# jenicek/mdir

Hardware: NVIDIA B200
Metric: queries/s vs 1M x 2048 db (70-query batches, top-100, fp32-faithful ranking) (higher is better)
Workload: dtype bf16

## Files before the change

include/mdir_b200.h:

```cpp
#ifndef MDIR_B200_H
#define MDIR_B200_H

#include <stddef.h>
#include <stdint.h>

#ifdef __cplusplus
extern "C" {
#endif

#define MDIR_ABI_VERSION 3

#define MDIR_E_ARG      (-1)
#define MDIR_E_DRIVER   (-2)
#define MDIR_E_DEVICE   (-3)

int         mdir_abi_version(void);
const char* mdir_last_error(void);
int         mdir_device_check(void);
uint64_t    mdir_launch_count(void);

#define MDIR_TUNE_SCAN_MAX_CTAS 1
#define MDIR_TUNE_FINALIZE_CLUSTER 2
#define MDIR_TUNE_FINALIZE_STAGE_CAP 3
int         mdir_tune(int key, int value);

#define MDIR_POOL_GEM  0
#define MDIR_POOL_MAC  1
#define MDIR_POOL_SPOC 2
int mdir_pool(int kind, const float* x, const int64_t* off, const int32_t* hw,
              int n_maps, int C, int hw_uniform, float p, float eps,
              float* out, void* stream);

int mdir_l2n(const float* x, int N, int C, int inner, float eps, float* out, void* stream);

int mdir_ms_aggregate(const float* pooled, int n_img, int S, int C, float l2n_eps,
                      float msp, const float* m, float* out, void* stream);

int mdir_whiten_project(const float* v, const float* m, int n, int D, const float* P, int dims,
                        float renorm_eps, float* out, void* stream);

size_t mdir_whiten_tc_workspace_bytes(int n, int D, int dims);
int mdir_whiten_project_tc(const float* v, const float* m, int n, int D, const float* Px3, int dims,
                           float renorm_eps, float* out, void* ws, void* stream);

typedef struct {
    int64_t src_off;
    int64_t dst_off;
    int32_t H, W;
    int32_t src_pitch;
    int32_t dst_pitch;
} mdir_image_desc;
size_t mdir_clahe_workspace_bytes(int n_img, int tiles_x, int tiles_y);
int mdir_clahe_u8(const uint8_t* src, uint8_t* dst, const mdir_image_desc* descs,
                  int n_img, int max_H, int max_W, double clip, int tiles_x, int tiles_y,
                  void* ws, void* stream);

typedef struct {
    int64_t rgb_off;
    int64_t out_off;
    int64_t l_off;
    int32_t H, W;
} mdir_rgb_desc;
int mdir_rgb_to_l_u8(const float* rgb, const mdir_rgb_desc* descs, int n_img, int64_t max_pixels,
                     const int16_t* lut, uint8_t* l_out, void* stream);
int mdir_lab_clahe_to_rgb(const float* rgb, const mdir_rgb_desc* descs, int n_img, int64_t max_pixels,
                          const int16_t* lut, const float* gamma_tab, const uint8_t* l_in, float* out,
                          void* stream);

int mdir_pack_bf16(const float* src, int64_t n, int D, int src_is_Dxn, uint16_t* dst, void* stream);

#define MDIR_SCAN_DENSE  0
#define MDIR_SCAN_SAMPLE 1
#define MDIR_SCAN_FILTER 2
#define MDIR_SCAN_TILE_ROWS 256
#define MDIR_CAND_SEGS 149
int mdir_sim_scan_bf16(const uint16_t* db, int64_t n_db, const uint16_t* q, int n_q, int D,
                       int mode, int sample_stride, int n_sample,
                       float* dense_out, int64_t dense_ld,
                       const uint64_t* tau, uint32_t idx_base,
                       uint64_t* cand, uint32_t* seg_counts, int cap_s, int cap_l, void* stream);

int mdir_sim_scan_dense_bf16(const uint16_t* db, int64_t n_db, const uint16_t* q, int n_q, int D,
                             float* dense_out, int64_t dense_ld, void* stream);

int mdir_sim_scan_wide_bf16(const uint16_t* db, int64_t n_db, const uint16_t* q, int n_q, int D, int mode,
                            int sample_stride, int n_sample, float* dense_out, int64_t dense_ld,
                            const uint64_t* tau, uint32_t idx_base, uint64_t* cand, uint32_t* seg_counts,
                            int cap_s, int cap_l, void* stream);

size_t mdir_sim_scan_fused_workspace_bytes(int n_q);
int mdir_sim_scan_fused_bf16(const uint16_t* db, int64_t n_db, const uint16_t* q, int n_q, int D,
                             int kth, uint64_t* tau, uint32_t idx_base,
                             uint64_t* cand, uint32_t* seg_counts, int cap_s, int cap_l,
                             void* ws, void* stream);

int mdir_sim_scan_fused_i8(const int8_t* db8, const float* row_scale, int64_t n_db, const int8_t* q8,
                           const float* q_scale, int n_q, int D, int kth, uint64_t* tau, uint32_t idx_base,
                           uint64_t* cand, uint32_t* seg_counts, int cap_s, int cap_l,
                           void* ws, void* stream);

int mdir_sim_scan_tf32(const float* db, int64_t n_db, const float* q, int n_q, int D,
                       int mode, int sample_stride, int n_sample,
                       float* dense_out, int64_t dense_ld,
                       const uint64_t* tau, uint32_t idx_base,
                       uint64_t* cand, uint32_t* seg_counts, int cap_s, int cap_l, void* stream);
int mdir_split_tf32x3(const float* src, int64_t n, int D, int role, float* dst, void* stream);

int mdir_sim_scan_bf16_live(const uint16_t* db, int64_t n_db, const uint16_t* q, int n_q, int D,
                            int mode, int sample_stride, int n_sample,
                            float* dense_out, int64_t dense_ld,
                            const uint64_t* tau, uint32_t idx_base,
                            uint64_t* cand, uint32_t* seg_counts, int cap_s, int cap_l,
                            const uint32_t* live, void* stream);
int mdir_sim_scan_wide_bf16_live(const uint16_t* db, int64_t n_db, const uint16_t* q, int n_q, int D, int mode,
                                 int sample_stride, int n_sample, float* dense_out, int64_t dense_ld,
                                 const uint64_t* tau, uint32_t idx_base, uint64_t* cand, uint32_t* seg_counts,
                                 int cap_s, int cap_l, const uint32_t* live, void* stream);
int mdir_sim_scan_fused_bf16_live(const uint16_t* db, int64_t n_db, const uint16_t* q, int n_q, int D,
                                  int kth, uint64_t* tau, uint32_t idx_base,
                                  uint64_t* cand, uint32_t* seg_counts, int cap_s, int cap_l,
                                  void* ws, const uint32_t* live, void* stream);
int mdir_sim_scan_fused_i8_live(const int8_t* db8, const float* row_scale, int64_t n_db, const int8_t* q8,
                                const float* q_scale, int n_q, int D, int kth, uint64_t* tau, uint32_t idx_base,
                                uint64_t* cand, uint32_t* seg_counts, int cap_s, int cap_l,
                                void* ws, const uint32_t* live, void* stream);
int mdir_live_update(uint32_t* live, int64_t capacity, uint32_t idx_base, const int64_t* ids, int64_t n_ids,
                     int value, void* stream);

uint64_t mdir_make_key(float score, uint32_t index);
float    mdir_key_score(uint64_t key);

int mdir_select_kth(const float* scores, int64_t ld, int64_t n, int n_q, int kth,
                    int sample_stride, uint32_t idx_base,
                    uint64_t* tau, uint64_t* cand, int64_t cand_row, uint32_t* seg_counts, int n_seg,
                    int cap, int approx, void* stream);
int mdir_select_kth_live(const float* scores, int64_t ld, int64_t n, int n_q, int kth,
                         int sample_stride, uint32_t idx_base,
                         uint64_t* tau, uint64_t* cand, int64_t cand_row, uint32_t* seg_counts, int n_seg,
                         int cap, int approx, const uint32_t* live, void* stream);

int mdir_topk_finalize(const uint64_t* cand, int64_t cand_row, const uint32_t* seg_counts, int n_seg,
                       int cap0, int cap_l, int n_q, int k,
                       float* out_scores, int32_t* out_idx, uint64_t* out_keys,
                       uint64_t* tau, int32_t* overflow, void* stream);

int mdir_topk_finalize_rescore(const uint64_t* cand, int64_t cand_row, const uint32_t* seg_counts, int n_seg,
                               int cap0, int cap_l, int n_q, int shortlist, int k_out,
                               const float* db32, int64_t n_db, uint32_t idx_base, const float* q32, int D,
                               const float* db_stats,
                               float* out_scores, int32_t* out_idx, uint64_t* out_keys,
                               uint64_t* tau, int32_t* overflow, void* stream);
int mdir_topk_finalize_rescore_eps(const uint64_t* cand, int64_t cand_row, const uint32_t* seg_counts, int n_seg,
                                   int cap0, int cap_l, int n_q, int shortlist, int k_out,
                                   const float* db32, int64_t n_db, uint32_t idx_base, const float* q32, int D,
                                   const float* db_stats, const float* q_eps,
                                   float* out_scores, int32_t* out_idx, uint64_t* out_keys,
                                   uint64_t* tau, int32_t* overflow, void* stream);
#define MDIR_STATUS_OVERFLOW    1
#define MDIR_STATUS_UNCERTIFIED 2

int mdir_pack_stats(const float* db32, const uint16_t* db16, int64_t n, int D, float* stats, void* stream);

int mdir_pack_stats_i8(const float* db32, const uint16_t* db16, int64_t n, int D, float* stats,
                       int8_t* db8, float* row_scale, void* stream);

int mdir_pack_q_i8(const float* q32, int n_q, int D, const float* stats, int8_t* q8, float* q_scale,
                   float* q_eps, void* stream);

int mdir_rescore_f32(const float* db32, int64_t n_db, uint32_t idx_base, const float* q32, int n_q, int D,
                     const int32_t* idx, int kk, uint64_t* out_keys, void* stream);

int mdir_qe_accumulate(const float* db32, int64_t n_db, uint32_t idx_base, int D, const int32_t* idx,
                       const float* scores, int n_q, int n_qe, float alpha, float* acc, void* stream);
int mdir_add_l2n(const float* a, const float* b, int n, int D, float* out, void* stream);

size_t mdir_rank_workspace_bytes(int64_t n_db, int n_q);
int mdir_rank_scores(const float* scores, int64_t n_db, int n_q, int query_major,
                     int64_t* ranks, int64_t ranks_ld, void* ws, void* stream);

size_t mdir_rank_fast_workspace_bytes(int64_t n_db, int n_q);
int mdir_rank_scores_fast(const float* scores, int64_t n_db, int n_q, int query_major,
                          int64_t* ranks, int64_t ranks_ld, void* ws, int32_t* status, void* stream);

size_t mdir_rank_hist_workspace_bytes(int64_t n_db, int n_q);
int mdir_rank_scores_hist(const float* scores, int64_t n_db, int n_q, int query_major,
                          int64_t* ranks, int64_t ranks_ld, void* ws, int32_t* status, void* stream);

size_t mdir_map_workspace_bytes(int64_t n_db, int n_q);
int mdir_compute_ap(const int64_t* ranks, int64_t n_db, int n_q, const int64_t* items, const int32_t* item_query,
                    const int32_t* item_class, int64_t n_items, const int32_t* n_pos, const int32_t* kappas,
                    int n_kappa, double* aps, double* prs, void* ws, void* stream);

int mdir_topk_plan(int64_t n_db, int kth, int sm_count, int* route, int* n_sample, int* stride);
size_t mdir_sim_topk_workspace_bytes(int D);
int mdir_sim_topk_bf16(const uint16_t* db16, const float* db32, const float* db_stats, int64_t n_db,
                       const float* q32, int n_q, int D, int k, int shortlist, uint32_t idx_base, int route,
                       float* out_scores, int32_t* out_idx, uint64_t* out_keys, int32_t* overflow,
                       void* ws, void* stream);
size_t mdir_gem_head_workspace_bytes(int n_img, int S, int C, int dims);
int mdir_gem_head(int kind, const float* x, const int64_t* off, const int32_t* hw, int n_img, int S, int C,
                  int hw_uniform, float p, float eps, float msp, const float* m, const float* P,
                  const float* Px3, int dims, float* out, void* ws, void* stream);

size_t mdir_shard_mailbox_bytes(int world, int max_q, int max_k);
int mdir_p2p_alloc(size_t bytes, void** ptr, void* handle64);
int mdir_p2p_open(const void* handle64, void** ptr);
int mdir_p2p_close(void* ptr);
int mdir_p2p_free(void* ptr);
#define MDIR_EXCHANGE_SYNC 0
#define MDIR_EXCHANGE_DEFERRED 1
#define MDIR_EXCHANGE_FLUSH 2
int mdir_shard_exchange_merge(const uint64_t* local_keys, int n_q, int k, int rank, int world,
                              int max_q, int max_k, int mode, void* const* mailboxes,
                              float* out_scores, int32_t* out_idx,
                              const int32_t* local_status, int32_t* out_status, void* stream);
int mdir_shard_status(const void* own_mailbox, int* status);

int mdir_mine_negatives(const int64_t* ranks, int64_t ranks_ld, int64_t n_pool, int n_q,
                        const int32_t* pool_cluster, const int32_t* q_cluster, int nnum,
                        int64_t* out_pos, int32_t* out_found, void* stream);
int mdir_pair_l2dist(const float* q, const float* pool, const int64_t* pos, int n_q, int nnum, int D,
                     float eps, float* out, void* stream);

size_t mdir_gemm_f64_workspace_bytes(int M, int N, int64_t K);
int mdir_gemm_f64(const double* A, int64_t lda, const double* a_sub, const double* B, int64_t ldb,
                  const double* b_sub, int b_is_kxn, int M, int N, int64_t K, double alpha,
                  double* C, int64_t ldc, void* ws, void* stream);
int mdir_pair_diff_f64(const double* X, int64_t ldx, int D, int64_t n_cols, const int64_t* qidx,
                       const int64_t* pidx, int64_t n_pairs, double* out, void* stream);
int mdir_cols_mean_f64(const double* X, int64_t ldx, int D, int64_t n_cols, const int64_t* idx,
                       int64_t n_idx, double* mean, void* stream);
int mdir_f32_to_f64(const float* src, int64_t n, double* dst, void* stream);

#ifdef __cplusplus
}
#endif
#endif
```

mdir_b200/_lib.py:

```python
import ctypes as C
import os

_HERE = os.path.dirname(os.path.abspath(__file__))
LIB_PATH = os.path.join(_HERE, "libmdir_b200.so")
_lib = None
ABI_VERSION = 3


class ImageDesc(C.Structure):
    _fields_ = [("src_off", C.c_int64), ("dst_off", C.c_int64), ("H", C.c_int32), ("W", C.c_int32),
                ("src_pitch", C.c_int32), ("dst_pitch", C.c_int32)]


_vp, _i, _i64, _f, _d, _u32, _u64, _sz = C.c_void_p, C.c_int, C.c_int64, C.c_float, C.c_double, C.c_uint32, C.c_uint64, C.c_size_t

PROTOTYPES = {
    "mdir_abi_version": (_i, []),
    "mdir_last_error": (C.c_char_p, []),
    "mdir_device_check": (_i, []),
    "mdir_launch_count": (_u64, []),
    "mdir_tune": (_i, [_i, _i]),
    "mdir_pool": (_i, [_i, _vp, _vp, _vp, _i, _i, _i, _f, _f, _vp, _vp]),
    "mdir_l2n": (_i, [_vp, _i, _i, _i, _f, _vp, _vp]),
    "mdir_ms_aggregate": (_i, [_vp, _i, _i, _i, _f, _f, _vp, _vp, _vp]),
    "mdir_whiten_project": (_i, [_vp, _vp, _i, _i, _vp, _i, _f, _vp, _vp]),
    "mdir_whiten_tc_workspace_bytes": (_sz, [_i, _i, _i]),
    "mdir_whiten_project_tc": (_i, [_vp, _vp, _i, _i, _vp, _i, _f, _vp, _vp, _vp]),
    "mdir_clahe_workspace_bytes": (_sz, [_i, _i, _i]),
    "mdir_clahe_u8": (_i, [_vp, _vp, _vp, _i, _i, _i, _d, _i, _i, _vp, _vp]),
    "mdir_rgb_to_l_u8": (_i, [_vp, _vp, _i, _i64, _vp, _vp, _vp]),
    "mdir_lab_clahe_to_rgb": (_i, [_vp, _vp, _i, _i64, _vp, _vp, _vp, _vp, _vp]),
    "mdir_pack_bf16": (_i, [_vp, _i64, _i, _i, _vp, _vp]),
    "mdir_sim_scan_bf16": (_i, [_vp, _i64, _vp, _i, _i, _i, _i, _i, _vp, _i64, _vp, _u32, _vp, _vp, _i, _i, _vp]),
    "mdir_sim_scan_dense_bf16": (_i, [_vp, _i64, _vp, _i, _i, _vp, _i64, _vp]),
    "mdir_sim_scan_wide_bf16": (_i, [_vp, _i64, _vp, _i, _i, _i, _i, _i, _vp, _i64, _vp, _u32, _vp, _vp, _i, _i, _vp]),
    "mdir_sim_scan_fused_workspace_bytes": (_sz, [_i]),
    "mdir_sim_scan_fused_bf16": (_i, [_vp, _i64, _vp, _i, _i, _i, _vp, _u32, _vp, _vp, _i, _i, _vp, _vp]),
    "mdir_sim_scan_fused_i8": (_i, [_vp, _vp, _i64, _vp, _vp, _i, _i, _i, _vp, _u32, _vp, _vp, _i, _i, _vp, _vp]),
    "mdir_sim_scan_tf32": (_i, [_vp, _i64, _vp, _i, _i, _i, _i, _i, _vp, _i64, _vp, _u32, _vp, _vp, _i, _i, _vp]),
    "mdir_split_tf32x3": (_i, [_vp, _i64, _i, _i, _vp, _vp]),
    "mdir_sim_scan_bf16_live": (_i, [_vp, _i64, _vp, _i, _i, _i, _i, _i, _vp, _i64, _vp, _u32, _vp, _vp, _i, _i, _vp, _vp]),
    "mdir_sim_scan_wide_bf16_live": (_i, [_vp, _i64, _vp, _i, _i, _i, _i, _i, _vp, _i64, _vp, _u32, _vp, _vp, _i, _i, _vp, _vp]),
    "mdir_sim_scan_fused_bf16_live": (_i, [_vp, _i64, _vp, _i, _i, _i, _vp, _u32, _vp, _vp, _i, _i, _vp, _vp, _vp]),
    "mdir_sim_scan_fused_i8_live": (_i, [_vp, _vp, _i64, _vp, _vp, _i, _i, _i, _vp, _u32, _vp, _vp, _i, _i, _vp, _vp, _vp]),
    "mdir_live_update": (_i, [_vp, _i64, _u32, _vp, _i64, _i, _vp]),
    "mdir_make_key": (_u64, [_f, _u32]),
    "mdir_key_score": (_f, [_u64]),
    "mdir_select_kth": (_i, [_vp, _i64, _i64, _i, _i, _i, _u32, _vp, _vp, _i64, _vp, _i, _i, _i, _vp]),
    "mdir_select_kth_live": (_i, [_vp, _i64, _i64, _i, _i, _i, _u32, _vp, _vp, _i64, _vp, _i, _i, _i, _vp, _vp]),
    "mdir_topk_finalize": (_i, [_vp, _i64, _vp, _i, _i, _i, _i, _i, _vp, _vp, _vp, _vp, _vp, _vp]),
    "mdir_topk_finalize_rescore": (_i, [_vp, _i64, _vp, _i, _i, _i, _i, _i, _i, _vp, _i64, _u32, _vp, _i, _vp, _vp, _vp, _vp, _vp, _vp, _vp]),
    "mdir_topk_finalize_rescore_eps": (_i, [_vp, _i64, _vp, _i, _i, _i, _i, _i, _i, _vp, _i64, _u32, _vp, _i, _vp, _vp, _vp, _vp, _vp, _vp, _vp, _vp]),
    "mdir_pack_stats": (_i, [_vp, _vp, _i64, _i, _vp, _vp]),
    "mdir_pack_stats_i8": (_i, [_vp, _vp, _i64, _i, _vp, _vp, _vp, _vp]),
    "mdir_pack_q_i8": (_i, [_vp, _i, _i, _vp, _vp, _vp, _vp, _vp]),
    "mdir_rescore_f32": (_i, [_vp, _i64, _u32, _vp, _i, _i, _vp, _i, _vp, _vp]),
    "mdir_qe_accumulate": (_i, [_vp, _i64, _u32, _i, _vp, _vp, _i, _i, _f, _vp, _vp]),
    "mdir_add_l2n": (_i, [_vp, _vp, _i, _i, _vp, _vp]),
    "mdir_map_workspace_bytes": (_sz, [_i64, _i]),
    "mdir_compute_ap": (_i, [_vp, _i64, _i, _vp, _vp, _vp, _i64, _vp, _vp, _i, _vp, _vp, _vp, _vp]),
    "mdir_topk_plan": (_i, [_i64, _i, _i, _vp, _vp, _vp]),
    "mdir_sim_topk_workspace_bytes": (_sz, [_i]),
    "mdir_sim_topk_bf16": (_i, [_vp, _vp, _vp, _i64, _vp, _i, _i, _i, _i, _u32, _i, _vp, _vp, _vp, _vp, _vp, _vp]),
    "mdir_gem_head_workspace_bytes": (_sz, [_i, _i, _i, _i]),
    "mdir_gem_head": (_i, [_i, _vp, _vp, _vp, _i, _i, _i, _i, _f, _f, _f, _vp, _vp, _vp, _i, _vp, _vp, _vp]),
    "mdir_shard_mailbox_bytes": (_sz, [_i, _i, _i]),
    "mdir_p2p_alloc": (_i, [_sz, _vp, _vp]),
    "mdir_p2p_open": (_i, [_vp, _vp]),
    "mdir_p2p_close": (_i, [_vp]),
    "mdir_p2p_free": (_i, [_vp]),
    "mdir_shard_exchange_merge": (_i, [_vp, _i, _i, _i, _i, _i, _i, _i, _vp, _vp, _vp, _vp, _vp, _vp]),
    "mdir_shard_status": (_i, [_vp, _vp]),
    "mdir_mine_negatives": (_i, [_vp, _i64, _i64, _i, _vp, _vp, _i, _vp, _vp, _vp]),
    "mdir_pair_l2dist": (_i, [_vp, _vp, _vp, _i, _i, _i, _f, _vp, _vp]),
    "mdir_gemm_f64_workspace_bytes": (_sz, [_i, _i, _i64]),
    "mdir_gemm_f64": (_i, [_vp, _i64, _vp, _vp, _i64, _vp, _i, _i, _i, _i64, _d, _vp, _i64, _vp, _vp]),
    "mdir_pair_diff_f64": (_i, [_vp, _i64, _i, _i64, _vp, _vp, _i64, _vp, _vp]),
    "mdir_cols_mean_f64": (_i, [_vp, _i64, _i, _i64, _vp, _i64, _vp, _vp]),
    "mdir_f32_to_f64": (_i, [_vp, _i64, _vp, _vp]),
    "mdir_rank_workspace_bytes": (_sz, [_i64, _i]),
    "mdir_rank_scores": (_i, [_vp, _i64, _i, _i, _vp, _i64, _vp, _vp]),
    "mdir_rank_fast_workspace_bytes": (_sz, [_i64, _i]),
    "mdir_rank_scores_fast": (_i, [_vp, _i64, _i, _i, _vp, _i64, _vp, _vp, _vp]),
    "mdir_rank_hist_workspace_bytes": (_sz, [_i64, _i]),
    "mdir_rank_scores_hist": (_i, [_vp, _i64, _i, _i, _vp, _i64, _vp, _vp, _vp]),
}


class MdirError(RuntimeError):
    pass


def lib():
    global _lib
    if _lib is None:
        if not os.path.exists(LIB_PATH):
            raise MdirError("%s is missing: run `python -m mdir_b200.build` (nvcc, sm_100a). "
                            "mdir_b200 has no CPU or PyTorch fallback." % LIB_PATH)
        l = C.CDLL(LIB_PATH)
        for name, (res, args) in PROTOTYPES.items():
            fn = getattr(l, name)
            fn.restype = res
            fn.argtypes = args
        if l.mdir_abi_version() != ABI_VERSION:
            raise MdirError("libmdir_b200.so ABI mismatch")
        _lib = l
    return _lib


def check(rc, what=""):
    if rc != 0:
        msg = lib().mdir_last_error()
        raise MdirError("%s failed (code %d): %s" % (what or "libmdir_b200 call", rc, (msg or b"").decode()))


def stream():
    import torch
    return C.c_void_p(torch.cuda.current_stream().cuda_stream)


def ptr(t):
    return C.c_void_p(t.data_ptr()) if t is not None else C.c_void_p(0)


def require_cuda(t, name="tensor"):
    if not t.is_cuda:
        raise MdirError("%s must live on a CUDA device (mdir_b200 has no CPU path); got %s" % (name, t.device))
    return t
```

mdir_b200/csrc/topk.cu:

```cuda
#include <cuda_bf16.h>

#include "common.cuh"

namespace mdir {

__device__ __forceinline__ uint32_t sample_pos_to_idx(int64_t i, int sample_stride, uint32_t idx_base) {
    if (sample_stride <= 1) return idx_base + (uint32_t)i;
    const int64_t j = i / MDIR_SCAN_TILE_ROWS, r = i - j * MDIR_SCAN_TILE_ROWS;
    return idx_base + (uint32_t)(j * sample_stride * MDIR_SCAN_TILE_ROWS + r);
}

__device__ __forceinline__ bool pos_live(const uint32_t* live, int64_t i, int sample_stride) {
    if (!live) return true;
    const uint32_t r = sample_pos_to_idx(i, sample_stride, 0u);
    return (__ldg(live + (r >> 5)) >> (r & 31)) & 1u;
}

__device__ __forceinline__ uint32_t block_kth_of_thread_values(uint32_t val, uint32_t kth, uint32_t* hist, uint32_t* s_prefix,
                                                               uint32_t* s_k) {
    const int lane = threadIdx.x & 31;
    __syncthreads();
    if (threadIdx.x == 0) { *s_prefix = 0u; *s_k = kth; }
    for (int pass = 0; pass < 4; ++pass) {
        const int shift = 24 - 8 * pass;
        if (threadIdx.x < 256) hist[threadIdx.x] = 0u;
        __syncthreads();
        const uint32_t prefix = *s_prefix;
        const uint32_t himask = pass == 0 ? 0u : (0xffffffffu << (shift + 8));
        const bool hit = (val & himask) == prefix;
        if (__any_sync(0xffffffffu, hit)) {
            const int d = (int)((val >> shift) & 0xffu);
            const unsigned peers = match_digit8(d, hit);
            if (hit && lane == (__ffs(peers) - 1)) atomicAdd(&hist[d], (uint32_t)__popc(peers));
        }
        __syncthreads();
        if (threadIdx.x < 32) {
            uint32_t before;
            const int b = find_bin_warp0(hist, *s_k, &before);
            if (lane == 0) {
                *s_k -= before;
                *s_prefix = prefix | ((uint32_t)b << shift);
            }
        }
        __syncthreads();
    }
    const uint32_t r = *s_prefix;
    __syncthreads();
    return r;
}

__global__ void __launch_bounds__(1024) select_kth_kernel(const float* __restrict__ scores, int64_t ld, int64_t n, int kth,
                                                          int sample_stride, uint32_t idx_base, uint64_t* __restrict__ tau,
                                                          uint64_t* __restrict__ cand, int64_t cand_row, uint32_t* __restrict__ seg_counts,
                                                          int n_seg, int cap, const uint32_t* __restrict__ live) {
    __shared__ uint32_t hist[256];
    __shared__ uint32_t s_prefix;
    __shared__ uint32_t s_k;
    __shared__ uint32_t s_n;
    __shared__ uint32_t s_ties;
    const int q = blockIdx.x;
    const int lane = threadIdx.x & 31;
    const float* sc = scores + (int64_t)q * ld;
    uint32_t result;
    uint32_t idx_limit = 0xffffffffu;
    const int64_t n_round = (n + 8191) & ~(int64_t)8191;
    if ((int64_t)kth > n) {
        result = 0xffffffffu;
    } else {
        uint32_t bound = 0xffffffffu;
        if (kth <= 1024) {
            uint32_t mymin = 0xffffffffu;
            for (int64_t base = 0; base < n_round; base += 8 * 1024) {
                float v[8];
#pragma unroll
                for (int u = 0; u < 8; ++u) {
                    const int64_t i = base + u * 1024 + threadIdx.x;
                    v[u] = i < n ? __ldg(sc + i) : 0.f;
                }
#pragma unroll
                for (int u = 0; u < 8; ++u) {
                    const int64_t i = base + u * 1024 + threadIdx.x;
                    if (i < n && pos_live(live, i, sample_stride)) mymin = min(mymin, desc_key(v[u]));
                }
            }
            bound = block_kth_of_thread_values(mymin, (uint32_t)kth, hist, &s_prefix, &s_k);
        }
        if (threadIdx.x == 0) { s_prefix = 0u; s_k = (uint32_t)kth; }
        for (int pass = 0; pass < 4; ++pass) {
            const int shift = 24 - 8 * pass;
            if (threadIdx.x < 256) hist[threadIdx.x] = 0u;
            __syncthreads();
            const uint32_t prefix = s_prefix;
            const uint32_t himask = pass == 0 ? 0u : (0xffffffffu << (shift + 8));
            for (int64_t base = 0; base < n_round; base += 8 * 1024) {
                float v[8];
#pragma unroll
                for (int u = 0; u < 8; ++u) {
                    const int64_t i = base + u * 1024 + threadIdx.x;
                    v[u] = i < n ? __ldg(sc + i) : 0.f;
                }
#pragma unroll
                for (int u = 0; u < 8; ++u) {
                    const int64_t i = base + u * 1024 + threadIdx.x;
                    const bool valid = i < n && pos_live(live, i, sample_stride);
                    const uint32_t key = desc_key(v[u]);
                    const bool hit = valid && key <= bound && ((key & himask) == prefix);
                    if (__any_sync(0xffffffffu, hit)) {
                        const int d = (int)((key >> shift) & 0xffu);
                        const unsigned peers = match_digit8(d, hit);
                        if (hit && lane == (__ffs(peers) - 1)) atomicAdd(&hist[d], (uint32_t)__popc(peers));
                    }
                }
            }
            __syncthreads();
            if (threadIdx.x < 32) {
                uint32_t before;
                const int b = find_bin_warp0(hist, s_k, &before);
                if (lane == 0) {
                    s_k -= before;
                    s_prefix = prefix | ((uint32_t)b << shift);
                    s_ties = hist[b];
                }
            }
            __syncthreads();
        }
        result = s_prefix;
        if (s_k < s_ties) {
            __syncthreads();
            if (threadIdx.x == 0) s_prefix = 0u;
            for (int pass = 0; pass < 4; ++pass) {
                const int shift = 24 - 8 * pass;
                if (threadIdx.x < 256) hist[threadIdx.x] = 0u;
                __syncthreads();
                const uint32_t prefix = s_prefix;
                const uint32_t himask = pass == 0 ? 0u : (0xffffffffu << (shift + 8));
                for (int64_t base = 0; base < n_round; base += 1024) {
                    const int64_t i = base + threadIdx.x;
                    const bool valid = i < n && pos_live(live, i, sample_stride);
                    const float v = valid ? __ldg(sc + i) : 0.f;
                    const uint32_t idx = sample_pos_to_idx(valid ? i : 0, sample_stride, idx_base);
                    const bool hit = valid && (desc_key(v) == result) && ((idx & himask) == prefix);
                    if (__any_sync(0xffffffffu, hit)) {
                        const int d = (int)((idx >> shift) & 0xffu);
                        const unsigned peers = match_digit8(d, hit);
                        if (hit && lane == (__ffs(peers) - 1)) atomicAdd(&hist[d], (uint32_t)__popc(peers));
                    }
                }
                __syncthreads();
                if (threadIdx.x < 32) {
                    uint32_t before;
                    const int b = find_bin_warp0(hist, s_k, &before);
                    if (lane == 0) {
                        s_k -= before;
                        s_prefix = prefix | ((uint32_t)b << shift);
                    }
                }
                __syncthreads();
            }
            idx_limit = s_prefix;
        }
    }
    const uint64_t tau_key = ((uint64_t)result << 32) | (uint64_t)idx_limit;
    __syncthreads();
    if (threadIdx.x == 0) { tau[q] = tau_key; s_n = 0u; }
    if (cand) {
        __syncthreads();
        for (int64_t base = 0; base < n_round; base += 8 * 1024) {
            float v[8];
#pragma unroll
            for (int u = 0; u < 8; ++u) {
                const int64_t i = base + u * 1024 + threadIdx.x;
                v[u] = i < n ? __ldg(sc + i) : -INFINITY;
            }
#pragma unroll
            for (int u = 0; u < 8; ++u) {
                const int64_t i = base + u * 1024 + threadIdx.x;
                if (i < n && desc_key(v[u]) <= result && pos_live(live, i, sample_stride)) {
                    const uint64_t key = make_key(v[u], sample_pos_to_idx(i, sample_stride, idx_base));
                    if (key <= tau_key) {
                        const uint32_t pos = atomicAdd(&s_n, 1u);
                        if (pos < (uint32_t)cap) cand[(int64_t)q * cand_row + pos] = key;
                    }
                }
            }
        }
        __syncthreads();
        if (threadIdx.x == 0) seg_counts[(int64_t)q * n_seg] = s_n;
        for (int sg = 1 + threadIdx.x; sg < n_seg; sg += blockDim.x) seg_counts[(int64_t)q * n_seg + sg] = 0u;
    }
}

__global__ void __launch_bounds__(1024, 1) select_kth_reg_kernel(const float* __restrict__ scores, int64_t ld, int n, int kth,
                                                                 int sample_stride, uint32_t idx_base, uint64_t* __restrict__ tau,
                                                                 uint64_t* __restrict__ cand, int64_t cand_row,
                                                                 uint32_t* __restrict__ seg_counts, int n_seg, int cap, int approx,
                                                                 const uint32_t* __restrict__ live) {
    __shared__ uint32_t hist[256];
    __shared__ uint32_t s_prefix, s_k, s_n, s_ties;
    const int q = blockIdx.x;
    const int lane = threadIdx.x & 31;
    const float* sc = scores + (int64_t)q * ld;
    uint32_t key[32];
#pragma unroll
    for (int u = 0; u < 32; ++u) {
        const int i = u * 1024 + threadIdx.x;
        key[u] = i < n && pos_live(live, i, sample_stride) ? desc_key(__ldg(sc + i)) : 0xffffffffu;
    }
    auto valid = [&](int u) { return live ? key[u] != 0xffffffffu : u * 1024 + (int)threadIdx.x < n; };
    uint32_t result = 0xffffffffu, idx_limit = 0xffffffffu;
    if (kth <= n) {
        uint32_t bound = 0xffffffffu;
        if (kth <= 1024) {
            uint32_t mymin = 0xffffffffu;
#pragma unroll
            for (int u = 0; u < 32; ++u)
                if (valid(u)) mymin = min(mymin, key[u]);
            bound = block_kth_of_thread_values(mymin, (uint32_t)kth, hist, &s_prefix, &s_k);
        }
        const bool use_bound = approx && kth <= 1024;
        if (threadIdx.x == 0) { s_prefix = use_bound ? bound : 0u; s_k = use_bound ? 0u : (uint32_t)kth; s_ties = 0u; }
        if (use_bound) __syncthreads();
        for (int pass = 0; pass < (use_bound ? 0 : 4); ++pass) {
            const int shift = 24 - 8 * pass;
            if (threadIdx.x < 256) hist[threadIdx.x] = 0u;
            __syncthreads();
            const uint32_t prefix = s_prefix;
            const uint32_t himask = pass == 0 ? 0u : (0xffffffffu << (shift + 8));
#pragma unroll
            for (int u = 0; u < 32; ++u) {
                const bool hit = valid(u) && key[u] <= bound && ((key[u] & himask) == prefix);
                if (__any_sync(0xffffffffu, hit)) {
                    const int d = (int)((key[u] >> shift) & 0xffu);
                    const unsigned peers = match_digit8(d, hit);
                    if (hit && lane == (__ffs(peers) - 1)) atomicAdd(&hist[d], (uint32_t)__popc(peers));
                }
            }
            __syncthreads();
            if (threadIdx.x < 32) {
                uint32_t before;
                const int b = find_bin_warp0(hist, s_k, &before);
                if (lane == 0) {
                    s_k -= before;
                    s_prefix = prefix | ((uint32_t)b << shift);
                    s_ties = hist[b];
                }
            }
            __syncthreads();
        }
        result = s_prefix;
        if (s_k < s_ties) {
            __syncthreads();
            if (threadIdx.x == 0) s_prefix = 0u;
            for (int pass = 0; pass < 4; ++pass) {
                const int shift = 24 - 8 * pass;
                if (threadIdx.x < 256) hist[threadIdx.x] = 0u;
                __syncthreads();
                const uint32_t prefix = s_prefix;
                const uint32_t himask = pass == 0 ? 0u : (0xffffffffu << (shift + 8));
#pragma unroll
                for (int u = 0; u < 32; ++u) {
                    const int i = u * 1024 + threadIdx.x;
                    const uint32_t idx = sample_pos_to_idx(i, sample_stride, idx_base);
                    const bool hit = valid(u) && key[u] == result && ((idx & himask) == prefix);
                    if (__any_sync(0xffffffffu, hit)) {
                        const int d = (int)((idx >> shift) & 0xffu);
                        const unsigned peers = match_digit8(d, hit);
                        if (hit && lane == (__ffs(peers) - 1)) atomicAdd(&hist[d], (uint32_t)__popc(peers));
                    }
                }
                __syncthreads();
                if (threadIdx.x < 32) {
                    uint32_t before;
                    const int b = find_bin_warp0(hist, s_k, &before);
                    if (lane == 0) {
                        s_k -= before;
                        s_prefix = prefix | ((uint32_t)b << shift);
                    }
                }
                __syncthreads();
            }
            idx_limit = s_prefix;
        }
    }
    const uint64_t tau_key = ((uint64_t)result << 32) | (uint64_t)idx_limit;
    __syncthreads();
    if (threadIdx.x == 0) { tau[q] = tau_key; s_n = 0u; }
    if (cand) {
        __syncthreads();
#pragma unroll
        for (int u = 0; u < 32; ++u) {
            const int i = u * 1024 + threadIdx.x;
            if (valid(u) && key[u] <= result) {
                const uint64_t k64 = ((uint64_t)key[u] << 32) | (uint64_t)sample_pos_to_idx(i, sample_stride, idx_base);
                if (k64 <= tau_key) {
                    const uint32_t pos = atomicAdd(&s_n, 1u);
                    if (pos < (uint32_t)cap) cand[(int64_t)q * cand_row + pos] = k64;
                }
            }
        }
        __syncthreads();
        if (threadIdx.x == 0) seg_counts[(int64_t)q * n_seg] = s_n;
        for (int sg = 1 + threadIdx.x; sg < n_seg; sg += blockDim.x) seg_counts[(int64_t)q * n_seg + sg] = 0u;
    }
}

__device__ __forceinline__ uint32_t cluster_ctarank() {
    uint32_t r;
    asm volatile("mov.u32 %0, %%cluster_ctarank;" : "=r"(r));
    return r;
}
__device__ __forceinline__ void cluster_sync_all() {
    asm volatile("barrier.cluster.arrive.release.aligned;\n\tbarrier.cluster.wait.acquire.aligned;" ::: "memory");
}
__device__ __forceinline__ uint32_t cluster_map(const void* p, uint32_t rank) {
    const uint32_t a = (uint32_t)__cvta_generic_to_shared(p);
    uint32_t r;
    asm volatile("mapa.shared::cluster.u32 %0, %1, %2;" : "=r"(r) : "r"(a), "r"(rank));
    return r;
}
__device__ __forceinline__ uint64_t cluster_ld_u64(uint32_t a) {
    uint64_t v;
    asm volatile("ld.shared::cluster.u64 %0, [%1];" : "=l"(v) : "r"(a) : "memory");
    return v;
}
__device__ __forceinline__ void cluster_st_u64(uint32_t a, uint64_t v) {
    asm volatile("st.shared::cluster.u64 [%0], %1;" ::"r"(a), "l"(v) : "memory");
}
__device__ __forceinline__ int cluster_ld_s32(uint32_t a) {
    int v;
    asm volatile("ld.shared::cluster.s32 %0, [%1];" : "=r"(v) : "r"(a) : "memory");
    return v;
}

__device__ __forceinline__ float rescore_row(const float* __restrict__ a, const float* qs, int D, int lane) {
    float acc = 0.f;
    if ((D & 3) == 0) {
        const float4* a4 = reinterpret_cast<const float4*>(a);
        const float4* b4 = reinterpret_cast<const float4*>(qs);
        const int n4 = D >> 2;
        float acc1 = 0.f, acc2 = 0.f, acc3 = 0.f;
        int i = lane;
        for (; i + 96 < n4; i += 128) {
            const float4 x0 = __ldg(a4 + i), x1 = __ldg(a4 + i + 32), x2 = __ldg(a4 + i + 64), x3 = __ldg(a4 + i + 96);
            const float4 y0 = b4[i], y1 = b4[i + 32], y2 = b4[i + 64], y3 = b4[i + 96];
            acc = fmaf(x0.x, y0.x, acc); acc = fmaf(x0.y, y0.y, acc); acc = fmaf(x0.z, y0.z, acc); acc = fmaf(x0.w, y0.w, acc);
            acc1 = fmaf(x1.x, y1.x, acc1); acc1 = fmaf(x1.y, y1.y, acc1); acc1 = fmaf(x1.z, y1.z, acc1); acc1 = fmaf(x1.w, y1.w, acc1);
            acc2 = fmaf(x2.x, y2.x, acc2); acc2 = fmaf(x2.y, y2.y, acc2); acc2 = fmaf(x2.z, y2.z, acc2); acc2 = fmaf(x2.w, y2.w, acc2);
            acc3 = fmaf(x3.x, y3.x, acc3); acc3 = fmaf(x3.y, y3.y, acc3); acc3 = fmaf(x3.z, y3.z, acc3); acc3 = fmaf(x3.w, y3.w, acc3);
        }
        for (; i < n4; i += 32) {
            const float4 x = __ldg(a4 + i), y = b4[i];
            acc = fmaf(x.x, y.x, acc); acc = fmaf(x.y, y.y, acc); acc = fmaf(x.z, y.z, acc); acc = fmaf(x.w, y.w, acc);
        }
        acc = (acc + acc1) + (acc2 + acc3);
    } else {
        for (int i = lane; i < D; i += 32) acc = fmaf(a[i], qs[i], acc);
    }
    return warp_sum(acc);
}

__device__ __forceinline__ bool topk_hist_select(uint64_t* skeys, int cnt, int k, int kpow2, uint64_t* out, uint32_t* hist, uint32_t* s_n,
                                                 uint32_t* scratch) {
    const int lane = threadIdx.x & 31, w = threadIdx.x >> 5;
    uint32_t mn = 0xffffffffu, mx = 0u;
    for (int i = threadIdx.x; i < cnt; i += blockDim.x) {
        const uint32_t h = (uint32_t)(skeys[i] >> 32);
        mn = min(mn, h);
        mx = max(mx, h);
    }
    mn = __reduce_min_sync(0xffffffffu, mn);
    mx = __reduce_max_sync(0xffffffffu, mx);
    if (lane == 0) { scratch[w] = mn; scratch[32 + w] = mx; }
    hist[threadIdx.x] = 0u;
    if (threadIdx.x == 0) *s_n = 0u;
    __syncthreads();
    mn = scratch[lane];
    mx = scratch[32 + lane];
    mn = __reduce_min_sync(0xffffffffu, mn);
    mx = __reduce_max_sync(0xffffffffu, mx);
    const float scale = 1024.0f / ((float)(mx - mn) + 1.0f);
    auto bin_of = [&](uint64_t key) { return min(1023, (int)((float)((uint32_t)(key >> 32) - mn) * scale)); };
    for (int i = threadIdx.x; i < cnt; i += blockDim.x) atomicAdd(&hist[bin_of(skeys[i])], 1u);
    __syncthreads();
    const uint32_t c = hist[threadIdx.x];
    uint32_t incl = c;
#pragma unroll
    for (int o = 1; o < 32; o <<= 1) {
        const uint32_t t = __shfl_up_sync(0xffffffffu, incl, o);
        if (lane >= o) incl += t;
    }
    __syncthreads();
    if (lane == 31) scratch[w] = incl;
    __syncthreads();
    uint32_t pre = 0;
    for (int j = 0; j < w; ++j) pre += scratch[j];
    incl += pre;
    if (incl >= (uint32_t)k && incl - c < (uint32_t)k) { scratch[32] = threadIdx.x; scratch[33] = incl; }
    if (threadIdx.x == 1023 && incl < (uint32_t)k) { scratch[32] = 1023u; scratch[33] = incl; }
    __syncthreads();
    const int b_star = (int)scratch[32];
    const int take = (int)scratch[33];
    if (take > 1024) return false;
    uint64_t* sel = skeys + cnt;
    for (int i = threadIdx.x; i < cnt; i += blockDim.x) {
        const uint64_t key = skeys[i];
        if (bin_of(key) <= b_star) sel[atomicAdd(s_n, 1u)] = key;
    }
    for (int i = threadIdx.x; i < kpow2; i += blockDim.x) out[i] = ~0ull;
    __syncthreads();
    if ((int)threadIdx.x < take) {
        const uint64_t mine = sel[threadIdx.x];
        int r = 0;
        for (int j = 0; j < take; ++j) r += sel[j] < mine ? 1 : 0;
        if (r < kpow2) out[r] = mine;
    }
    __syncthreads();
    return true;
}

__device__ __forceinline__ void rescore_row2(const float* __restrict__ a0, const float* __restrict__ a1, const float* qs, int D, int lane,
                                             float& r0, float& r1) {
    if ((D & 3) != 0) {
        r0 = rescore_row(a0, qs, D, lane);
        r1 = rescore_row(a1, qs, D, lane);
        return;
    }
    const float4* p0 = reinterpret_cast<const float4*>(a0);
    const float4* p1 = reinterpret_cast<const float4*>(a1);
    const float4* b4 = reinterpret_cast<const float4*>(qs);
    const int n4 = D >> 2;
    float s0a = 0.f, s0b = 0.f, s1a = 0.f, s1b = 0.f;
    int i = lane;
    for (; i + 96 < n4; i += 128) {
        const float4 x0 = __ldg(p0 + i), x1 = __ldg(p0 + i + 32), x2 = __ldg(p0 + i + 64), x3 = __ldg(p0 + i + 96);
        const float4 z0 = __ldg(p1 + i), z1 = __ldg(p1 + i + 32), z2 = __ldg(p1 + i + 64), z3 = __ldg(p1 + i + 96);
        float4 y = b4[i];
        s0a = fmaf(x0.x, y.x, s0a); s0a = fmaf(x0.y, y.y, s0a); s0a = fmaf(x0.z, y.z, s0a); s0a = fmaf(x0.w, y.w, s0a);
        s1a = fmaf(z0.x, y.x, s1a); s1a = fmaf(z0.y, y.y, s1a); s1a = fmaf(z0.z, y.z, s1a); s1a = fmaf(z0.w, y.w, s1a);
        y = b4[i + 32];
        s0b = fmaf(x1.x, y.x, s0b); s0b = fmaf(x1.y, y.y, s0b); s0b = fmaf(x1.z, y.z, s0b); s0b = fmaf(x1.w, y.w, s0b);
        s1b = fmaf(z1.x, y.x, s1b); s1b = fmaf(z1.y, y.y, s1b); s1b = fmaf(z1.z, y.z, s1b); s1b = fmaf(z1.w, y.w, s1b);
        y = b4[i + 64];
        s0a = fmaf(x2.x, y.x, s0a); s0a = fmaf(x2.y, y.y, s0a); s0a = fmaf(x2.z, y.z, s0a); s0a = fmaf(x2.w, y.w, s0a);
        s1a = fmaf(z2.x, y.x, s1a); s1a = fmaf(z2.y, y.y, s1a); s1a = fmaf(z2.z, y.z, s1a); s1a = fmaf(z2.w, y.w, s1a);
        y = b4[i + 96];
        s0b = fmaf(x3.x, y.x, s0b); s0b = fmaf(x3.y, y.y, s0b); s0b = fmaf(x3.z, y.z, s0b); s0b = fmaf(x3.w, y.w, s0b);
        s1b = fmaf(z3.x, y.x, s1b); s1b = fmaf(z3.y, y.y, s1b); s1b = fmaf(z3.z, y.z, s1b); s1b = fmaf(z3.w, y.w, s1b);
    }
    for (; i < n4; i += 32) {
        const float4 x = __ldg(p0 + i), z = __ldg(p1 + i), y = b4[i];
        s0a = fmaf(x.x, y.x, s0a); s0a = fmaf(x.y, y.y, s0a); s0a = fmaf(x.z, y.z, s0a); s0a = fmaf(x.w, y.w, s0a);
        s1a = fmaf(z.x, y.x, s1a); s1a = fmaf(z.y, y.y, s1a); s1a = fmaf(z.z, y.z, s1a); s1a = fmaf(z.w, y.w, s1a);
    }
    r0 = warp_sum(s0a + s0b);
    r1 = warp_sum(s1a + s1b);
}

template <int CS>
__device__ __forceinline__ void rescore_share(uint64_t* local_list, uint32_t remote_list, bool remote, int j0, int n, int crank,
                                              const float* __restrict__ db32, int64_t n_db, uint32_t idx_base, const float* qs, int D) {
    const int lane = threadIdx.x & 31;
    for (int j = (threadIdx.x >> 5) * CS + crank; j < n; j += 64 * CS) {
        const int jb = j + 32 * CS;
        const uint64_t key0 = remote ? cluster_ld_u64(remote_list + 8u * (uint32_t)(j0 + j)) : local_list[j0 + j];
        uint64_t key1 = ~0ull;
        if (jb < n) key1 = remote ? cluster_ld_u64(remote_list + 8u * (uint32_t)(j0 + jb)) : local_list[j0 + jb];
        const uint32_t g0 = (uint32_t)key0, g1 = (uint32_t)key1;
        const int64_t row0 = (int64_t)g0 - (int64_t)idx_base, row1 = (int64_t)g1 - (int64_t)idx_base;
        const bool ok0 = key0 != ~0ull && row0 >= 0 && row0 < n_db, ok1 = key1 != ~0ull && row1 >= 0 && row1 < n_db;
        float s0 = 0.f, s1 = 0.f;
        if (ok0 && ok1) rescore_row2(db32 + row0 * D, db32 + row1 * D, qs, D, lane, s0, s1);
        else if (ok0) s0 = rescore_row(db32 + row0 * D, qs, D, lane);
        else if (ok1) s1 = rescore_row(db32 + row1 * D, qs, D, lane);
        const uint64_t n0 = ok0 ? make_key(s0, g0) : ~0ull, n1 = ok1 ? make_key(s1, g1) : ~0ull;
        __syncwarp();
        if (lane == 0) {
            if (remote) {
                cluster_st_u64(remote_list + 8u * (uint32_t)(j0 + j), n0);
                if (jb < n) cluster_st_u64(remote_list + 8u * (uint32_t)(j0 + jb), n1);
            } else {
                local_list[j0 + j] = n0;
                if (jb < n) local_list[j0 + jb] = n1;
            }
        }
    }
}

template <int CS>
__global__ void __launch_bounds__(1024) topk_finalize_kernel(const uint64_t* __restrict__ cand, int64_t cand_row,
                                                             const uint32_t* __restrict__ seg_counts, int n_seg, int cap0, int cap_l,
                                                             int k, int smem_cap, int sl_cap, float* __restrict__ out_scores,
                                                             int32_t* __restrict__ out_idx, uint64_t* __restrict__ out_keys,
                                                             uint64_t* __restrict__ tau, int32_t* __restrict__ overflow,
                                                             const float* __restrict__ db32, int64_t n_db, uint32_t idx_base,
                                                             const float* __restrict__ q32, int D, int k_out,
                                                             const float* __restrict__ db_stats, const float* __restrict__ q_eps) {
    extern __shared__ uint64_t skeys[];
    __shared__ uint32_t hist[256];
    __shared__ uint64_t s_prefix;
    __shared__ uint32_t s_k, s_done, s_out;
    __shared__ int s_off[MDIR_CAND_SEGS + 1];
    __shared__ int s_ovf;
    __shared__ int s_hdr[3];
    __shared__ uint64_t s_tkey;
    __shared__ float s_red[96];
    __shared__ uint32_t hist_sel[1024];
    uint64_t* sorted = skeys + smem_cap;
    const int q = blockIdx.x / CS;
    const int crank = CS > 1 ? (int)cluster_ctarank() : 0;
    const int lane = threadIdx.x & 31;
    int kpow2 = 32;
    while (kpow2 < k) kpow2 <<= 1;
    if (CS > 1 && crank != 0) {
        float* qs = reinterpret_cast<float*>(sorted + sl_cap);
        for (int i = threadIdx.x; i < D; i += blockDim.x) qs[i] = q32[(int64_t)q * D + i];
        __syncthreads();
        cluster_sync_all();
        const int nk = cluster_ld_s32(cluster_map(&s_hdr[0], 0));
        const int off = cluster_ld_s32(cluster_map(&s_hdr[1], 0));
        const uint32_t rk0 = cluster_map(skeys + off, 0);
        rescore_share<CS>(nullptr, rk0, true, 0, nk, crank, db32, n_db, idx_base, qs, D);
        cluster_sync_all();
        cluster_sync_all();
        const int n_ext = cluster_ld_s32(cluster_map(&s_hdr[2], 0));
        rescore_share<CS>(nullptr, rk0, true, nk, n_ext, crank, db32, n_db, idx_base, qs, D);
        cluster_sync_all();
        return;
    }
    const uint64_t tau_in = tau ? tau[q] : ~0ull;
    if (threadIdx.x < 32) {
        constexpr int kRounds = (MDIR_CAND_SEGS + 31) / 32;
        uint32_t raw[kRounds];
#pragma unroll
        for (int i = 0; i < kRounds; ++i) {
            const int sg = i * 32 + lane;
            raw[i] = sg < n_seg ? seg_counts[(int64_t)q * n_seg + sg] : 0u;
        }
        int run = 0, ovf = 0;
#pragma unroll
        for (int i = 0; i < kRounds; ++i) {
            const int sg = i * 32 + lane;
            int c = 0;
            if (sg < n_seg) {
                const uint32_t cp = (uint32_t)(sg == 0 ? cap0 : cap_l);
                if (raw[i] > cp) ovf = 1;
                c = (int)min(raw[i], cp);
            }
            int incl = c;
#pragma unroll
            for (int o = 1; o < 32; o <<= 1) {
                const int t = __shfl_up_sync(0xffffffffu, incl, o);
                if (lane >= o) incl += t;
            }
            if (sg < n_seg) s_off[sg] = run + incl - c;
            run += __shfl_sync(0xffffffffu, incl, 31);
        }
        ovf = __any_sync(0xffffffffu, ovf);
        if (lane == 0) { s_off[n_seg] = run; s_ovf = ovf; }
    }
    __syncthreads();
    const int total = s_off[n_seg];
    const int cnt = min(total, smem_cap);
    const bool ovf_any = s_ovf || total > smem_cap;
    {
        const uint64_t* row = cand + (int64_t)q * cand_row;
        for (int p = threadIdx.x; p < cnt; p += blockDim.x) {
            int lo = 0, hi = n_seg;
            while (hi - lo > 1) {
                const int mid = (lo + hi) >> 1;
                if (s_off[mid] <= p) lo = mid; else hi = mid;
            }
            const int64_t base = lo == 0 ? 0 : (int64_t)cap0 + (int64_t)(lo - 1) * cap_l;
            skeys[p] = row[base + (p - s_off[lo])];
        }
    }
    __syncthreads();
    const uint64_t* res;
    int nres;
    if (cnt > k + 96 && cnt + 1024 <= smem_cap &&
        topk_hist_select(skeys, cnt, k, kpow2, sorted, hist_sel, &s_out, reinterpret_cast<uint32_t*>(s_red))) {
        res = sorted;
        nres = min(cnt, k);
    } else if (cnt <= 1024 && cnt + kpow2 <= smem_cap) {
        uint64_t mine = ~0ull;
        int r = 0;
        if ((int)threadIdx.x < cnt) {
            mine = skeys[threadIdx.x];
            for (int j = 0; j < cnt; ++j) r += skeys[j] < mine ? 1 : 0;
        }
        __syncthreads();
        if ((int)threadIdx.x < cnt) skeys[r] = mine;
        for (int i = cnt + threadIdx.x; i < cnt + kpow2 && i < smem_cap; i += blockDim.x) skeys[i] = ~0ull;
        __syncthreads();
        res = skeys;
        nres = cnt;
    } else if (cnt <= 2 * kpow2 || cnt <= 1024) {
        int n = 32;
        while (n < cnt) n <<= 1;
        for (int i = cnt + threadIdx.x; i < n; i += blockDim.x) skeys[i] = ~0ull;
        __syncthreads();
        bitonic_sort_smem(skeys, n);
        res = skeys;
        nres = cnt;
    } else {
        if (threadIdx.x == 0) { s_prefix = 0ull; s_k = (uint32_t)k; s_done = 0u; s_out = 0u; }
        __syncthreads();
        const int cnt_round = (cnt + 1023) & ~1023;
        uint64_t thresh = ~0ull;
        for (int pass = 0; pass < 8; ++pass) {
            const int shift = 56 - 8 * pass;
            if (threadIdx.x < 256) hist[threadIdx.x] = 0u;
            __syncthreads();
            const uint64_t prefix = s_prefix;
            const uint64_t himask = pass == 0 ? 0ull : (~0ull << (shift + 8));
            for (int i = threadIdx.x; i < cnt_round; i += 1024) {
                const bool valid = i < cnt;
                const uint64_t key = valid ? skeys[i] : 0ull;
                const bool hit = valid && ((key & himask) == prefix);
                if (__any_sync(0xffffffffu, hit)) {
                    const int d = (int)((key >> shift) & 0xffu);
                    const unsigned peers = match_digit8(d, hit);
                    if (hit && lane == (__ffs(peers) - 1)) atomicAdd(&hist[d], (uint32_t)__popc(peers));
                }
            }
            __syncthreads();
            if (threadIdx.x < 32) {
                uint32_t before;
                const int b = find_bin_warp0(hist, s_k, &before);
                if (lane == 0) {
                    const uint32_t need = s_k - before;
                    s_k = need;
                    s_prefix = prefix | ((uint64_t)b << shift);
                    if (need == hist[b] || shift == 0) s_done = 1u;
                }
            }
            __syncthreads();
            if (s_done) {
                thresh = s_prefix | (shift ? ((1ull << shift) - 1ull) : 0ull);
                break;
            }
        }
        for (int i = threadIdx.x; i < kpow2; i += blockDim.x) sorted[i] = ~0ull;
        __syncthreads();
        for (int i = threadIdx.x; i < cnt; i += blockDim.x) {
            const uint64_t key = skeys[i];
            if (key <= thresh) {
                const uint32_t pos = atomicAdd(&s_out, 1u);
                if (pos < (uint32_t)kpow2) sorted[pos] = key;
            }
        }
        __syncthreads();
        bitonic_sort_smem(sorted, kpow2);
        res = sorted;
        nres = min(cnt, k);
    }
    int status = ovf_any ? 1 : 0;
    if (threadIdx.x == 0 && ovf_any && tau && nres > 0) tau[q] = res[min(k, nres) - 1];
    int k_emit = k;
    if (db32) {
        uint64_t* sl = sorted;
        float* qs = reinterpret_cast<float*>(sorted + sl_cap);
        const int nk = min(k, nres);
        if (res != sl) {
            for (int j = threadIdx.x; j < nk; j += blockDim.x) sl[j] = res[j];
        }
        float q2 = 0.f, qt2 = 0.f, qf2 = 0.f;
        for (int i = threadIdx.x; i < D; i += blockDim.x) {
            const float v = q32[(int64_t)q * D + i];
            qs[i] = v;
            const float vt = __bfloat162float(__float2bfloat16_rn(v));
            q2 = fmaf(v, v, q2);
            qt2 = fmaf(vt, vt, qt2);
            qf2 = fmaf(v - vt, v - vt, qf2);
        }
        if (threadIdx.x == 0) { s_hdr[0] = nk; s_hdr[1] = (int)(sl - skeys); s_hdr[2] = 0; s_out = 0u; s_tkey = ~0ull; }
        __syncthreads();
        const uint64_t last16 = nk > 0 ? sl[nk - 1] : 0ull;
        float eps = 0.f;
        if (db_stats && q_eps) {
            eps = q_eps[q];
        } else if (db_stats) {
            q2 = warp_sum(q2); qt2 = warp_sum(qt2); qf2 = warp_sum(qf2);
            const int wi = threadIdx.x >> 5;
            if (lane == 0) { s_red[wi] = q2; s_red[32 + wi] = qt2; s_red[64 + wi] = qf2; }
            __syncthreads();
            q2 = warp_sum(s_red[lane]); qt2 = warp_sum(s_red[32 + lane]); qf2 = warp_sum(s_red[64 + lane]);
            const float e_max = sqrtf(db_stats[0]), x_max = sqrtf(db_stats[1]);
            eps = e_max * sqrtf(qt2) + x_max * sqrtf(qf2) + 1.25f * (float)D * 5.9604645e-8f * x_max * sqrtf(q2);
            eps = eps * 1.001f + 1e-7f;
        }
        __syncthreads();
        if (CS > 1) cluster_sync_all();
        rescore_share<CS>(sl, 0u, false, 0, nk, 0, db32, n_db, idx_base, qs, D);
        if (CS > 1) cluster_sync_all();
        __syncthreads();
        int n_ext = 0;
        if (db_stats) {
            if (nk >= k_out) {
                if (nk <= 1024) {
                    if ((int)threadIdx.x < nk) {
                        const uint64_t mine = sl[threadIdx.x];
                        int r = 0;
                        for (int j = 0; j < nk; ++j) {
                            const uint64_t o = sl[j];
                            r += (o < mine || (o == mine && j < (int)threadIdx.x)) ? 1 : 0;
                        }
                        if (r == k_out - 1) s_tkey = mine;
                    }
                } else {
                    for (int j = nk + threadIdx.x; j < kpow2; j += blockDim.x) sl[j] = ~0ull;
                    __syncthreads();
                    bitonic_sort_smem(sl, kpow2);
                    if (threadIdx.x == 0) s_tkey = sl[k_out - 1];
                }
            }
            __syncthreads();
            const uint64_t tkey = s_tkey;
            const uint64_t bound = tkey == ~0ull ? ~0ull : ((uint64_t)desc_key(key_score(tkey) - eps) << 32) | 0xffffffffull;
            const int ext_cap = sl_cap - nk;
            for (int i = threadIdx.x; i < cnt; i += blockDim.x) {
                const uint64_t key = skeys[i];
                if (key > last16 && key <= bound && key != ~0ull) {
                    const uint32_t pos = atomicAdd(&s_out, 1u);
                    if (pos < (uint32_t)ext_cap) sl[nk + pos] = key;
                }
            }
            __syncthreads();
            n_ext = min((int)s_out, ext_cap);
            if ((int)s_out > ext_cap || bound > tau_in || ovf_any) status |= 2;
            if (threadIdx.x == 0) s_hdr[2] = n_ext;
            __syncthreads();
        }
        if (CS > 1) cluster_sync_all();
        rescore_share<CS>(sl, 0u, false, nk, n_ext, 0, db32, n_db, idx_base, qs, D);
        if (CS > 1) cluster_sync_all();
        __syncthreads();
        const int n_all = nk + n_ext;
        if (n_all <= 1024) {
            if ((int)threadIdx.x < n_all) {
                const uint64_t mine = sl[threadIdx.x];
                int r = 0;
                for (int j = 0; j < n_all; ++j) {
                    const uint64_t o = sl[j];
                    r += (o < mine || (o == mine && j < (int)threadIdx.x)) ? 1 : 0;
                }
                skeys[r] = mine;
            }
            __syncthreads();
            res = skeys;
        } else {
            int n = 32;
            while (n < n_all) n <<= 1;
            for (int j = n_all + threadIdx.x; j < n; j += blockDim.x) sl[j] = ~0ull;
            __syncthreads();
            bitonic_sort_smem(sl, n);
            res = sl;
        }
        nres = n_all;
        k_emit = k_out;
    }
    if (threadIdx.x == 0 && overflow) overflow[q] = status;
    for (int j = threadIdx.x; j < k_emit; j += blockDim.x) {
        const uint64_t key = j < nres ? res[j] : ~0ull;
        const bool ok = j < nres && key != ~0ull;
        if (out_scores) out_scores[(int64_t)q * k_emit + j] = ok ? key_score(key) : -INFINITY;
        if (out_idx) out_idx[(int64_t)q * k_emit + j] = ok ? (int32_t)(uint32_t)key : -1;
        if (out_keys) out_keys[(int64_t)q * k_emit + j] = ok ? key : ~0ull;
    }
}

__global__ void __launch_bounds__(256) rescore_f32_kernel(const float* __restrict__ db32, int64_t n_db, uint32_t idx_base,
                                                          const float* __restrict__ q32, int n_q, int D,
                                                          const int32_t* __restrict__ idx, int kk, uint64_t* __restrict__ out_keys) {
    const int lane = threadIdx.x & 31;
    const int64_t item = (int64_t)blockIdx.x * (blockDim.x >> 5) + (threadIdx.x >> 5);
    if (item >= (int64_t)n_q * kk) return;
    const int q = (int)(item / kk);
    const int32_t gi = idx[item];
    const int64_t row = (int64_t)(uint32_t)gi - (int64_t)idx_base;
    if (gi < 0 || row < 0 || row >= n_db) {
        if (lane == 0) out_keys[item] = ~0ull;
        return;
    }
    const float* a = db32 + row * D;
    const float* b = q32 + (int64_t)q * D;
    float acc = 0.f;
    if ((D & 3) == 0) {
        const float4* a4 = reinterpret_cast<const float4*>(a);
        const float4* b4 = reinterpret_cast<const float4*>(b);
        for (int i = lane; i < (D >> 2); i += 32) {
            const float4 x = a4[i], y = b4[i];
            acc = fmaf(x.x, y.x, acc); acc = fmaf(x.y, y.y, acc); acc = fmaf(x.z, y.z, acc); acc = fmaf(x.w, y.w, acc);
        }
    } else {
        for (int i = lane; i < D; i += 32) acc = fmaf(a[i], b[i], acc);
    }
    acc = warp_sum(acc);
    if (lane == 0) out_keys[item] = make_key(acc, (uint32_t)gi);
}

__global__ void __launch_bounds__(256) pack_bf16_rows_kernel(const float* __restrict__ src, int64_t total, __nv_bfloat16* __restrict__ dst) {
    const int64_t i = ((int64_t)blockIdx.x * blockDim.x + threadIdx.x) * 4;
    if (i + 3 < total) {
        const float4 v = *reinterpret_cast<const float4*>(src + i);
        __nv_bfloat162 lo = __floats2bfloat162_rn(v.x, v.y), hi = __floats2bfloat162_rn(v.z, v.w);
        uint2 o;
        o.x = *reinterpret_cast<uint32_t*>(&lo);
        o.y = *reinterpret_cast<uint32_t*>(&hi);
        *reinterpret_cast<uint2*>(dst + i) = o;
    } else {
        for (int64_t j = i; j < total; ++j) dst[j] = __float2bfloat16_rn(src[j]);
    }
}

__global__ void __launch_bounds__(256) pack_bf16_transpose_kernel(const float* __restrict__ src, int64_t n, int D,
                                                                  __nv_bfloat16* __restrict__ dst) {
    __shared__ float tile[32][33];
    const int64_t n0 = (int64_t)blockIdx.x * 32;
    const int d0 = blockIdx.y * 32;
    const int tx = threadIdx.x & 31, ty = threadIdx.x >> 5;
    for (int r = ty; r < 32; r += 8) {
        const int d = d0 + r;
        const int64_t i = n0 + tx;
        tile[r][tx] = (d < D && i < n) ? src[(int64_t)d * n + i] : 0.f;
    }
    __syncthreads();
    for (int r = ty; r < 32; r += 8) {
        const int64_t i = n0 + r;
        const int d = d0 + tx;
        if (i < n && d < D) dst[i * D + d] = __float2bfloat16_rn(tile[tx][r]);
    }
}

__global__ void __launch_bounds__(256) qe_accumulate_kernel(const float* __restrict__ db32, int64_t n_db, uint32_t idx_base, int D,
                                                            const int32_t* __restrict__ idx, const float* __restrict__ scores,
                                                            int n_qe, float alpha, float* __restrict__ acc) {
    __shared__ float w_s[256];
    __shared__ int64_t row_s[256];
    const int q = blockIdx.x;
    for (int j = threadIdx.x; j < n_qe; j += blockDim.x) {
        const int32_t gi = idx[(int64_t)q * n_qe + j];
        const int64_t row = (int64_t)(uint32_t)gi - (int64_t)idx_base;
        const bool own = gi >= 0 && row >= 0 && row < n_db;
        row_s[j] = own ? row : -1;
        w_s[j] = own ? powf(fmaxf(scores[(int64_t)q * n_qe + j], 0.f), alpha) : 0.f;
    }
    __syncthreads();
    for (int d = threadIdx.x; d < D; d += blockDim.x) {
        float a = 0.f;
        for (int j = 0; j < n_qe; ++j)
            if (row_s[j] >= 0) a = fmaf(w_s[j], db32[row_s[j] * D + d], a);
        acc[(int64_t)q * D + d] = a;
    }
}

__global__ void __launch_bounds__(256) add_l2n_kernel(const float* a, const float* b, int D, float* out) {
    __shared__ float red[32];
    const int n = blockIdx.x;
    float s = 0.f;
    for (int d = threadIdx.x; d < D; d += blockDim.x) {
        const float v = a[(int64_t)n * D + d] + (b ? b[(int64_t)n * D + d] : 0.f);
        s += v * v;
    }
    s = block_sum(s, red);
    const float inv = 1.0f / sqrtf(s);
    for (int d = threadIdx.x; d < D; d += blockDim.x)
        out[(int64_t)n * D + d] = (a[(int64_t)n * D + d] + (b ? b[(int64_t)n * D + d] : 0.f)) * inv;
}

}

using namespace mdir;

extern "C" uint64_t mdir_make_key(float score, uint32_t index) { return make_key(score, index); }
extern "C" float mdir_key_score(uint64_t key) { return key_score(key); }

extern "C" int mdir_select_kth_live(const float* scores, int64_t ld, int64_t n, int n_q, int kth, int sample_stride,
                                    uint32_t idx_base, uint64_t* tau, uint64_t* cand, int64_t cand_row, uint32_t* seg_counts, int n_seg,
                                    int cap, int approx, const uint32_t* live, void* stream) {
    MDIR_CHECK_ARG(scores && tau && n >= 0 && n_q >= 0 && kth >= 1 && ld >= n);
    MDIR_CHECK_ARG(cand == nullptr || (seg_counts != nullptr && cap >= 1 && n_seg >= 1 && cand_row >= cap));
    if (n_q == 0) return 0;
    if (n <= 32 * 1024) {
        select_kth_reg_kernel<<<n_q, 1024, 0, (cudaStream_t)stream>>>(scores, ld, (int)n, kth, sample_stride, idx_base, tau, cand,
                                                                      cand_row, seg_counts, n_seg, cap, approx, live);
        MDIR_LAUNCH_CHECK();
        return 0;
    }
    select_kth_kernel<<<n_q, 1024, 0, (cudaStream_t)stream>>>(scores, ld, n, kth, sample_stride, idx_base, tau, cand, cand_row,
                                                              seg_counts, n_seg, cap, live);
    MDIR_LAUNCH_CHECK();
    return 0;
}

extern "C" int mdir_select_kth(const float* scores, int64_t ld, int64_t n, int n_q, int kth, int sample_stride,
                               uint32_t idx_base, uint64_t* tau, uint64_t* cand, int64_t cand_row, uint32_t* seg_counts, int n_seg,
                               int cap, int approx, void* stream) {
    return mdir_select_kth_live(scores, ld, n, n_q, kth, sample_stride, idx_base, tau, cand, cand_row, seg_counts, n_seg, cap, approx,
                                nullptr, stream);
}

namespace mdir {
__global__ void __launch_bounds__(256) live_update_kernel(uint32_t* __restrict__ live, int64_t capacity, uint32_t idx_base,
                                                          const int64_t* __restrict__ ids, int64_t n_ids, int value) {
    const int64_t i = (int64_t)blockIdx.x * blockDim.x + threadIdx.x;
    if (i >= n_ids) return;
    const int64_t r = ids[i] - (int64_t)idx_base;
    if (r < 0 || r >= capacity) return;
    const uint32_t bit = 1u << (uint32_t)(r & 31);
    if (value) atomicOr(live + (r >> 5), bit);
    else atomicAnd(live + (r >> 5), ~bit);
}
}

extern "C" int mdir_live_update(uint32_t* live, int64_t capacity, uint32_t idx_base, const int64_t* ids, int64_t n_ids, int value,
                                void* stream) {
    MDIR_CHECK_ARG(live && capacity >= 0 && n_ids >= 0 && (ids || n_ids == 0));
    if (n_ids == 0) return 0;
    MDIR_CHECK_ARG((n_ids + 255) / 256 <= 0x7fffffff);
    live_update_kernel<<<(unsigned)((n_ids + 255) / 256), 256, 0, (cudaStream_t)stream>>>(live, capacity, idx_base, ids, n_ids, value);
    MDIR_LAUNCH_CHECK();
    return 0;
}

static int launch_finalize(const uint64_t* cand, int64_t cand_row, const uint32_t* seg_counts, int n_seg, int cap0, int cap_l, int n_q,
                           int k, float* out_scores, int32_t* out_idx, uint64_t* out_keys, uint64_t* tau, int32_t* overflow,
                           const float* db32, int64_t n_db, uint32_t idx_base, const float* q32, int D, int k_out, const float* db_stats,
                           void* stream, const float* q_eps = nullptr) {
    MDIR_CHECK_ARG(cand && seg_counts && n_seg >= 1 && n_seg <= MDIR_CAND_SEGS && cap0 >= 0 && n_q >= 0 && k >= 1 && k <= 4096);
    MDIR_CHECK_ARG(n_seg == 1 || cap_l >= 1);
    MDIR_CHECK_ARG(cand_row >= (int64_t)cap0 + (int64_t)(n_seg - 1) * cap_l);
    if (n_q == 0) return 0;
    int kpow2 = 32;
    while (kpow2 < k) kpow2 <<= 1;
    int64_t want = (int64_t)cap0 + (int64_t)(n_seg - 1) * cap_l;
    int smem_cap = 1024;
    while (smem_cap < want && smem_cap < 16384) smem_cap <<= 1;
    if (g_finalize_stage_cap > 0 && smem_cap > g_finalize_stage_cap) smem_cap = g_finalize_stage_cap;
    if (smem_cap < 2 * kpow2) smem_cap = 2 * kpow2;
    int sl_cap = db32 ? 2 * kpow2 : kpow2;
    if (db32 && q_eps) {
        const int64_t want = (int64_t)kpow2 + n_db / 512;
        while (sl_cap < want && sl_cap < 2048) sl_cap <<= 1;
    }
    size_t smem = (size_t)(smem_cap + sl_cap) * 8;
    if (db32) {
        MDIR_CHECK_ARG(q32 && D > 0 && D <= 8192 && k_out >= 1 && k_out <= k && n_db >= 0);
        MDIR_CHECK_ARG((((uintptr_t)db32 | (uintptr_t)q32) & 15) == 0);
        MDIR_CHECK_ARG(db_stats == nullptr || tau != nullptr);
        smem += (size_t)D * 4;
    }
    constexpr int kFinalizeMaxSmem = 232448 - 7424;
    MDIR_CHECK_ARG(smem <= (size_t)kFinalizeMaxSmem);
    static PerDeviceOnce once;
    if (once.first() != 0) {
        const int max_smem = kFinalizeMaxSmem;
        MDIR_CUDA(cudaFuncSetAttribute(topk_finalize_kernel<1>, cudaFuncAttributeMaxDynamicSharedMemorySize, max_smem));
        MDIR_CUDA(cudaFuncSetAttribute(topk_finalize_kernel<2>, cudaFuncAttributeMaxDynamicSharedMemorySize, max_smem));
    }
    const int sm_count = device_sm_count();
    if (db32 && g_finalize_cluster && 2 * n_q <= sm_count) {
        cudaLaunchConfig_t cfg = {};
        cfg.gridDim = dim3(2 * n_q);
        cfg.blockDim = dim3(1024);
        cfg.dynamicSmemBytes = smem;
        cfg.stream = (cudaStream_t)stream;
        cudaLaunchAttribute attr[1];
        attr[0].id = cudaLaunchAttributeClusterDimension;
        attr[0].val.clusterDim.x = 2;
        attr[0].val.clusterDim.y = 1;
        attr[0].val.clusterDim.z = 1;
        cfg.attrs = attr;
        cfg.numAttrs = 1;
        MDIR_CUDA(cudaLaunchKernelEx(&cfg, topk_finalize_kernel<2>, cand, cand_row, seg_counts, n_seg, cap0, cap_l, k, smem_cap, sl_cap, out_scores,
                                     out_idx, out_keys, tau, overflow, db32, n_db, idx_base, q32, D, k_out, db_stats, q_eps));
        MDIR_LAUNCH_CHECK();
        return 0;
    }
    topk_finalize_kernel<1><<<n_q, 1024, smem, (cudaStream_t)stream>>>(cand, cand_row, seg_counts, n_seg, cap0, cap_l, k, smem_cap, sl_cap,
                                                                        out_scores, out_idx, out_keys, tau, overflow, db32, n_db, idx_base,
                                                                        q32, D, k_out, db_stats, q_eps);
    MDIR_LAUNCH_CHECK();
    return 0;
}

extern "C" int mdir_topk_finalize(const uint64_t* cand, int64_t cand_row, const uint32_t* seg_counts, int n_seg, int cap0, int cap_l,
                                  int n_q, int k, float* out_scores, int32_t* out_idx, uint64_t* out_keys, uint64_t* tau,
                                  int32_t* overflow, void* stream) {
    return launch_finalize(cand, cand_row, seg_counts, n_seg, cap0, cap_l, n_q, k, out_scores, out_idx, out_keys, tau, overflow, nullptr, 0,
                           0, nullptr, 0, 0, nullptr, stream);
}

extern "C" int mdir_topk_finalize_rescore(const uint64_t* cand, int64_t cand_row, const uint32_t* seg_counts, int n_seg, int cap0,
                                          int cap_l, int n_q, int shortlist, int k_out, const float* db32, int64_t n_db,
                                          uint32_t idx_base, const float* q32, int D, const float* db_stats, float* out_scores,
                                          int32_t* out_idx, uint64_t* out_keys, uint64_t* tau, int32_t* overflow, void* stream) {
    MDIR_CHECK_ARG(db32 != nullptr);
    return launch_finalize(cand, cand_row, seg_counts, n_seg, cap0, cap_l, n_q, shortlist, out_scores, out_idx, out_keys, tau, overflow,
                           db32, n_db, idx_base, q32, D, k_out, db_stats, stream);
}

extern "C" int mdir_topk_finalize_rescore_eps(const uint64_t* cand, int64_t cand_row, const uint32_t* seg_counts, int n_seg, int cap0,
                                              int cap_l, int n_q, int shortlist, int k_out, const float* db32, int64_t n_db,
                                              uint32_t idx_base, const float* q32, int D, const float* db_stats, const float* q_eps,
                                              float* out_scores, int32_t* out_idx, uint64_t* out_keys, uint64_t* tau, int32_t* overflow,
                                              void* stream) {
    MDIR_CHECK_ARG(db32 != nullptr && db_stats != nullptr && q_eps != nullptr);
    return launch_finalize(cand, cand_row, seg_counts, n_seg, cap0, cap_l, n_q, shortlist, out_scores, out_idx, out_keys, tau, overflow,
                           db32, n_db, idx_base, q32, D, k_out, db_stats, stream, q_eps);
}

namespace mdir {
__global__ void __launch_bounds__(256) pack_stats_kernel(const float* __restrict__ db32, const __nv_bfloat16* __restrict__ db16, int64_t n, int D,
                                                         uint32_t* __restrict__ stats) {
    const int lane = threadIdx.x & 31;
    const int64_t warps = (int64_t)gridDim.x * (blockDim.x >> 5);
    float e_max = 0.f, x_max = 0.f;
    for (int64_t r = (int64_t)blockIdx.x * (blockDim.x >> 5) + (threadIdx.x >> 5); r < n; r += warps) {
        const float* a = db32 + r * D;
        const __nv_bfloat16* b = db16 + r * D;
        float e2 = 0.f, x2 = 0.f;
        for (int i = lane; i < D; i += 32) {
            const float x = a[i];
            const float d = __bfloat162float(b[i]) - x;
            e2 = fmaf(d, d, e2);
            x2 = fmaf(x, x, x2);
        }
        e_max = fmaxf(e_max, warp_sum(e2));
        x_max = fmaxf(x_max, warp_sum(x2));
    }
    if (lane == 0) {
        atomicMax(&stats[0], __float_as_uint(e_max * 1.0001f));
        atomicMax(&stats[1], __float_as_uint(x_max * 1.0001f));
    }
}
}

extern "C" int mdir_pack_stats(const float* db32, const uint16_t* db16, int64_t n, int D, float* stats, void* stream) {
    MDIR_CHECK_ARG(db32 && db16 && stats && n >= 0 && D > 0);
    MDIR_CUDA(cudaMemsetAsync(stats, 0, 2 * sizeof(float), (cudaStream_t)stream));
    if (n == 0) return 0;
    const int64_t blocks = (n + 7) / 8;
    pack_stats_kernel<<<(unsigned)(blocks < 148 * 8 ? blocks : 148 * 8), 256, 0, (cudaStream_t)stream>>>(
        db32, reinterpret_cast<const __nv_bfloat16*>(db16), n, D, reinterpret_cast<uint32_t*>(stats));
    MDIR_LAUNCH_CHECK();
    return 0;
}

namespace mdir {
__device__ __forceinline__ float quant_i8(float v, float s) {
    return s > 0.f ? fminf(fmaxf(rintf(__fdiv_rn(v, s)), -127.f), 127.f) : 0.f;
}

__global__ void __launch_bounds__(256) pack_stats_i8_kernel(const float* __restrict__ db32, const __nv_bfloat16* __restrict__ db16, int64_t n,
                                                            int D, uint32_t* __restrict__ stats, int8_t* __restrict__ db8,
                                                            float* __restrict__ row_scale) {
    const int lane = threadIdx.x & 31;
    const int64_t warps = (int64_t)gridDim.x * (blockDim.x >> 5);
    float e_max = 0.f, x_max = 0.f, e8_max = 0.f, rel_max = 0.f;
    for (int64_t r = (int64_t)blockIdx.x * (blockDim.x >> 5) + (threadIdx.x >> 5); r < n; r += warps) {
        const float* a = db32 + r * D;
        const __nv_bfloat16* b = db16 + r * D;
        float e2 = 0.f, x2 = 0.f, m = 0.f;
        for (int i = lane; i < D; i += 32) {
            const float x = a[i];
            const float d = __bfloat162float(b[i]) - x;
            e2 = fmaf(d, d, e2);
            x2 = fmaf(x, x, x2);
            m = fmaxf(m, fabsf(x));
        }
        e2 = warp_sum(e2);
        x2 = warp_sum(x2);
        const float s = __fdiv_rn(warp_max(m), 127.f);
        float q2 = 0.f;
        for (int i = lane * 4; i < D; i += 128) {
            const float4 x = *reinterpret_cast<const float4*>(a + i);
            const float c0 = quant_i8(x.x, s), c1 = quant_i8(x.y, s), c2 = quant_i8(x.z, s), c3 = quant_i8(x.w, s);
            char4 o;
            o.x = (signed char)c0; o.y = (signed char)c1; o.z = (signed char)c2; o.w = (signed char)c3;
            *reinterpret_cast<char4*>(db8 + r * D + i) = o;
            const float d0 = fmaf(-s, c0, x.x), d1 = fmaf(-s, c1, x.y), d2 = fmaf(-s, c2, x.z), d3 = fmaf(-s, c3, x.w);
            q2 = fmaf(d0, d0, fmaf(d1, d1, fmaf(d2, d2, fmaf(d3, d3, q2))));
        }
        q2 = warp_sum(q2);
        if (lane == 0) row_scale[r] = s;
        e_max = fmaxf(e_max, e2);
        x_max = fmaxf(x_max, x2);
        e8_max = fmaxf(e8_max, q2);
        if (x2 > 0.f) rel_max = fmaxf(rel_max, q2 / x2);
    }
    if (lane == 0) {
        atomicMax(&stats[0], __float_as_uint(e_max * 1.0001f));
        atomicMax(&stats[1], __float_as_uint(x_max * 1.0001f));
        atomicMax(&stats[2], __float_as_uint(e8_max * 1.001f));
        atomicMax(&stats[3], __float_as_uint(rel_max * 1.001f));
    }
}

__global__ void __launch_bounds__(32) pack_q_i8_kernel(const float* __restrict__ q32, int n_q, int n_pad, int D, const float* __restrict__ stats,
                                                       int8_t* __restrict__ q8, float* __restrict__ q_scale, float* __restrict__ q_eps) {
    const int q = blockIdx.x, lane = threadIdx.x;
    int8_t* hi_row = q8 + (int64_t)q * D;
    int8_t* lo_row = q8 + (int64_t)(n_pad + q) * D;
    if (q >= n_q) {
        for (int i = lane * 4; i < D; i += 128) {
            *reinterpret_cast<char4*>(hi_row + i) = make_char4(0, 0, 0, 0);
            *reinterpret_cast<char4*>(lo_row + i) = make_char4(0, 0, 0, 0);
        }
        return;
    }
    const float* v = q32 + (int64_t)q * D;
    float m = 0.f, q2 = 0.f;
    for (int i = lane; i < D; i += 32) {
        const float x = v[i];
        m = fmaxf(m, fabsf(x));
        q2 = fmaf(x, x, q2);
    }
    const float s_hi = __fdiv_rn(warp_max(m), 127.f);
    float m2 = 0.f;
    for (int i = lane; i < D; i += 32) m2 = fmaxf(m2, fabsf(fmaf(-s_hi, quant_i8(v[i], s_hi), v[i])));
    const float s_lo = __fdiv_rn(warp_max(m2), 127.f);
    float h2 = 0.f, l2 = 0.f, qh2 = 0.f, d2 = 0.f;
    for (int i = lane * 4; i < D; i += 128) {
        const float4 x = *reinterpret_cast<const float4*>(v + i);
        const float xs[4] = {x.x, x.y, x.z, x.w};
        signed char ho[4], lo[4];
#pragma unroll
        for (int j = 0; j < 4; ++j) {
            const float h = quant_i8(xs[j], s_hi);
            const float r = fmaf(-s_hi, h, xs[j]);
            const float l = quant_i8(r, s_lo);
            const float d = fmaf(-s_lo, l, r);
            const float qh = fmaf(s_lo, l, s_hi * h);
            ho[j] = (signed char)h;
            lo[j] = (signed char)l;
            h2 = fmaf(h, h, h2);
            l2 = fmaf(l, l, l2);
            qh2 = fmaf(qh, qh, qh2);
            d2 = fmaf(d, d, d2);
        }
        *reinterpret_cast<char4*>(hi_row + i) = make_char4(ho[0], ho[1], ho[2], ho[3]);
        *reinterpret_cast<char4*>(lo_row + i) = make_char4(lo[0], lo[1], lo[2], lo[3]);
    }
    q2 = warp_sum(q2); h2 = warp_sum(h2); l2 = warp_sum(l2); qh2 = warp_sum(qh2); d2 = warp_sum(d2);
    if (lane == 0) {
        const float x_max = sqrtf(stats[1]), e8 = sqrtf(stats[2]);
        const float u = 5.9604645e-8f;
        float eps = e8 * sqrtf(qh2) + x_max * sqrtf(d2) + 1.25f * (float)D * u * x_max * sqrtf(q2) +
                    8.f * u * (x_max + e8) * (s_hi * sqrtf(h2) + s_lo * sqrtf(l2));
        q_scale[2 * q] = s_hi;
        q_scale[2 * q + 1] = s_lo;
        q_eps[q] = eps * 1.001f + 1e-7f;
    }
}
}

extern "C" int mdir_pack_stats_i8(const float* db32, const uint16_t* db16, int64_t n, int D, float* stats, int8_t* db8, float* row_scale,
                                  void* stream) {
    MDIR_CHECK_ARG(db32 && db16 && stats && db8 && row_scale && n >= 0 && D > 0 && D % 128 == 0);
    MDIR_CHECK_ARG((((uintptr_t)db32 | (uintptr_t)db8) & 15) == 0);
    MDIR_CUDA(cudaMemsetAsync(stats, 0, 4 * sizeof(float), (cudaStream_t)stream));
    if (n == 0) return 0;
    const int64_t blocks = (n + 7) / 8;
    pack_stats_i8_kernel<<<(unsigned)(blocks < 148 * 8 ? blocks : 148 * 8), 256, 0, (cudaStream_t)stream>>>(
        db32, reinterpret_cast<const __nv_bfloat16*>(db16), n, D, reinterpret_cast<uint32_t*>(stats), db8, row_scale);
    MDIR_LAUNCH_CHECK();
    return 0;
}

extern "C" int mdir_pack_q_i8(const float* q32, int n_q, int D, const float* stats, int8_t* q8, float* q_scale, float* q_eps, void* stream) {
    MDIR_CHECK_ARG(q32 && stats && q8 && q_scale && q_eps && n_q >= 1 && n_q <= 128 && D > 0 && D % 128 == 0);
    MDIR_CHECK_ARG((((uintptr_t)q32 | (uintptr_t)q8) & 15) == 0);
    const int n_pad = (n_q + 15) & ~15;
    pack_q_i8_kernel<<<n_pad, 32, 0, (cudaStream_t)stream>>>(q32, n_q, n_pad, D, stats, q8, q_scale, q_eps);
    MDIR_LAUNCH_CHECK();
    return 0;
}

extern "C" int mdir_rescore_f32(const float* db32, int64_t n_db, uint32_t idx_base, const float* q32, int n_q, int D,
                                const int32_t* idx, int kk, uint64_t* out_keys, void* stream) {
    MDIR_CHECK_ARG(db32 && q32 && idx && out_keys && n_db >= 0 && n_q >= 0 && D > 0 && kk >= 1);
    MDIR_CHECK_ARG((((uintptr_t)db32 | (uintptr_t)q32) & 15) == 0);
    const int64_t items = (int64_t)n_q * kk;
    if (items == 0) return 0;
    rescore_f32_kernel<<<(unsigned)((items + 7) / 8), 256, 0, (cudaStream_t)stream>>>(db32, n_db, idx_base, q32, n_q, D, idx, kk,
                                                                                      out_keys);
    MDIR_LAUNCH_CHECK();
    return 0;
}

extern "C" int mdir_pack_bf16(const float* src, int64_t n, int D, int src_is_Dxn, uint16_t* dst, void* stream) {
    MDIR_CHECK_ARG(src && dst && n >= 0 && D > 0);
    if (n == 0) return 0;
    cudaStream_t st = (cudaStream_t)stream;
    if (!src_is_Dxn) {
        MDIR_CHECK_ARG((((uintptr_t)src & 15) | ((uintptr_t)dst & 7)) == 0);
        const int64_t total = n * D;
        const int64_t threads = (total + 3) / 4;
        pack_bf16_rows_kernel<<<(unsigned)((threads + 255) / 256), 256, 0, st>>>(src, total, (__nv_bfloat16*)dst);
    } else {
        dim3 grid((unsigned)((n + 31) / 32), (unsigned)((D + 31) / 32));
        MDIR_CHECK_ARG(grid.y <= 65535);
        pack_bf16_transpose_kernel<<<grid, 256, 0, st>>>(src, n, D, (__nv_bfloat16*)dst);
    }
    MDIR_LAUNCH_CHECK();
    return 0;
}

extern "C" int mdir_qe_accumulate(const float* db32, int64_t n_db, uint32_t idx_base, int D, const int32_t* idx, const float* scores,
                                  int n_q, int n_qe, float alpha, float* acc, void* stream) {
    MDIR_CHECK_ARG(db32 && idx && scores && acc && n_db >= 0 && D > 0 && n_q >= 0 && n_qe >= 1 && n_qe <= 256);
    if (n_q == 0) return 0;
    qe_accumulate_kernel<<<n_q, 256, 0, (cudaStream_t)stream>>>(db32, n_db, idx_base, D, idx, scores, n_qe, alpha, acc);
    MDIR_LAUNCH_CHECK();
    return 0;
}

extern "C" int mdir_add_l2n(const float* a, const float* b, int n, int D, float* out, void* stream) {
    MDIR_CHECK_ARG(a && out && n >= 0 && D > 0);
    if (n == 0) return 0;
    add_l2n_kernel<<<n, 256, 0, (cudaStream_t)stream>>>(a, b, D, out);
    MDIR_LAUNCH_CHECK();
    return 0;
}
```

mdir_b200/search.py:

```python
import contextlib

import numpy as np
import torch

from . import _lib

TILE = 256
MAX_Q = 128
DENSE_LAUNCH_Q = 1 << 20
MAX_Q_WIDE = 256
SINGLE_GPU_SCAN_CTAS = 140
WIDE_Q = 1024
N_SEGS = 149
CAP_S = 8192
CAP_L = 96
CAND_ROW = CAP_S + 148 * CAP_L
STAGE_CAP = 16384
MAX_SAMPLE_TILES = 512
FUSED_CAP_L = CAND_ROW // 148
TARGET_CAND = 4500


STATUS_OVERFLOW, STATUS_UNCERTIFIED, STATUS_PEER_TIMEOUT = 1, 2, 4
MAX_KTH = 4096
I8_MAX_REL_RESIDUAL = 0.02
I8_MIN_ROWS = 900000


def default_shortlist(k):
    return -(-(-(-5 * int(k) // 4)) // 64) * 64


def balanced_grid(n_work, max_ctas):
    if n_work <= 0 or max_ctas <= 0:
        return 1
    if n_work <= max_ctas:
        return int(n_work)
    rounds = -(-n_work // max_ctas)
    return int(-(-n_work // rounds))


def _as_dev_f32(x, device):
    if isinstance(x, np.ndarray):
        x = torch.from_numpy(np.ascontiguousarray(x, dtype=np.float32))
    if x.dtype != torch.float32:
        x = x.float()
    if x.device != device:
        x = x.pin_memory().to(device, non_blocking=True) if x.device.type == "cpu" else x.to(device)
    return x.contiguous()


def pack_bf16(x, dxn=False, out=None):
    _lib.require_cuda(x, "descriptors")
    x = x.contiguous()
    if dxn:
        D, n = x.shape
    else:
        n, D = x.shape
    if D % 8:
        raise _lib.MdirError("descriptor dimension must be a multiple of 8 (got %d)" % D)
    if out is None:
        out = torch.empty((n, D), dtype=torch.bfloat16, device=x.device)
    with torch.cuda.device(x.device):
        _lib.check(_lib.lib().mdir_pack_bf16(_lib.ptr(x), n, D, 1 if dxn else 0, _lib.ptr(out), _lib.stream()), "mdir_pack_bf16")
    return out


def check_ids(ids, lo, hi):
    if isinstance(ids, torch.Tensor):
        ids = ids.detach().cpu().numpy()
    a = np.asarray(ids)
    if a.size and not np.issubdtype(a.dtype, np.integer):
        raise _lib.MdirError("ids must be integers (got %s)" % a.dtype)
    a = a.astype(np.int64).ravel()
    bad = (a < lo) | (a >= hi)
    if bad.any():
        raise _lib.MdirError("id %d is outside this index's ids [%d, %d)" % (int(a[bad][0]), lo, hi))
    return a - lo


def ids_for_rank(ids, ranges, rank):
    if isinstance(ids, torch.Tensor):
        ids = ids.detach().cpu().numpy()
    a = np.asarray(ids)
    if a.size and not np.issubdtype(a.dtype, np.integer):
        raise _lib.MdirError("ids must be integers (got %s)" % a.dtype)
    a = a.astype(np.int64).ravel()
    owned = np.zeros(a.shape, dtype=bool)
    for lo, hi in ranges:
        owned |= (a >= lo) & (a < hi)
    if not owned.all():
        raise _lib.MdirError("id %d is outside every shard of this index" % int(a[~owned][0]))
    lo, hi = ranges[rank]
    return a[(a >= lo) & (a < hi)]


class Index:

    fused = True
    certify = True
    _sms = None

    def __init__(self, vecs, dxn=False, device="cuda", keep_fp32=True, idx_base=0, capacity=None):
        self.device = torch.device(device)
        if self.device.type != "cuda":
            raise _lib.MdirError("Index needs a CUDA device (no CPU path)")
        v = _as_dev_f32(vecs, self.device)
        n, D = (v.shape[1], v.shape[0]) if dxn else (v.shape[0], v.shape[1])
        cap = n if capacity is None else int(capacity)
        if cap < n:
            raise _lib.MdirError("capacity %d is smaller than the %d rows given" % (cap, n))
        if int(idx_base) < 0 or int(idx_base) + cap > 1 << 32:
            raise _lib.MdirError("idx_base + capacity must stay within [0, 2**32]")
        with torch.cuda.device(self.device):
            db16 = torch.zeros((cap, D), dtype=torch.bfloat16, device=self.device) if cap > n else None
            self.db16 = pack_bf16(v, dxn=dxn, out=db16)
            self.n, self.D = self.db16.shape
            self.idx_base = int(idx_base)
            self.db32 = None
            if keep_fp32:
                if cap == n:
                    self.db32 = v.t().contiguous() if dxn else v
                else:
                    self.db32 = torch.zeros((cap, D), dtype=torch.float32, device=self.device)
                    self.db32[:n].copy_(v.t() if dxn else v)
            self._init_live(n)
        self._ws = {}
        self._stats = None
        self.db8 = self.row_scale = None
        self.route = None
        self.cert = {"queries": 0, "flagged": 0, "widened_blocks": 0, "uncertified": 0, "int8_blocks": 0, "int8_redone": 0}

    @classmethod
    def from_packed(cls, db16, db32=None, idx_base=0):
        self = cls.__new__(cls)
        self.device = db16.device
        self.db16 = db16
        self.n, self.D = db16.shape
        self.db32 = db32
        self.idx_base = int(idx_base)
        with torch.cuda.device(self.device):
            self._init_live(self.n)
        self._ws = {}
        self._stats = None
        self.db8 = self.row_scale = None
        self.route = None
        self.cert = {"queries": 0, "flagged": 0, "widened_blocks": 0, "uncertified": 0, "int8_blocks": 0, "int8_redone": 0}
        return self

    def _init_live(self, n_used):
        words = -(-self.n // TILE) * (TILE // 32)
        bits = np.zeros(words * 32, dtype=bool)
        bits[:n_used] = True
        host = np.packbits(bits, bitorder="little").view("<u4").view(np.int32)
        self.live = torch.from_numpy(host.copy()).to(self.device)
        self._live_host = bits[:self.n].copy()
        self._n_used = int(n_used)

    @property
    def n_live(self):
        return int(self._live_host.sum())

    def _require_all_live(self, what):
        if self.n_live != self.n:
            raise _lib.MdirError("%s scores every slot and does not support an index with removed rows or free capacity "
                                 "(%d of %d slots live); use search()" % (what, self.n_live, self.n))

    def _set_live(self, rows, value):
        rows = np.unique(rows)
        rows = rows[self._live_host[rows] != bool(value)]
        if rows.size == 0:
            return
        ids = torch.from_numpy(rows + self.idx_base).to(self.device)
        _lib.check(_lib.lib().mdir_live_update(_lib.ptr(self.live), self.n, self.idx_base, _lib.ptr(ids), int(rows.size), int(value),
                                               _lib.stream()), "mdir_live_update")
        self._live_host[rows] = bool(value)

    def remove(self, ids):
        rows = check_ids(ids, self.idx_base, self.idx_base + self.n)
        with torch.cuda.device(self.device):
            self._set_live(rows, 0)

    def restore(self, ids):
        rows = check_ids(ids, self.idx_base, self.idx_base + self.n)
        if rows.size and int(rows.max()) >= self._n_used:
            raise _lib.MdirError("id %d names a slot that was never filled" % (int(rows.max()) + self.idx_base))
        with torch.cuda.device(self.device):
            self._set_live(rows, 1)

    def add(self, vecs):
        lib = _lib.lib()
        with torch.cuda.device(self.device):
            v = _as_dev_f32(vecs, self.device)
            if v.dim() != 2 or v.shape[1] != self.D:
                raise _lib.MdirError("add() expects (m, %d) rows, got %s" % (self.D, tuple(v.shape)))
            m, s0 = int(v.shape[0]), self._n_used
            if s0 + m > self.n:
                raise _lib.MdirError("index is full: %d free slots, %d rows given" % (self.n - s0, m))
            if m == 0:
                return torch.empty((0,), dtype=torch.int64)
            s1 = s0 + m
            pack_bf16(v, out=self.db16[s0:s1])
            if self.db32 is not None:
                self.db32[s0:s1].copy_(v)
            if self._stats is not None:
                st = torch.zeros((4,), dtype=torch.float32, device=self.device)
                if self.db8 is not None:
                    _lib.check(lib.mdir_pack_stats_i8(_lib.ptr(self.db32[s0:s1]), _lib.ptr(self.db16[s0:s1]), m, self.D, _lib.ptr(st),
                                                      _lib.ptr(self.db8[s0:s1]), _lib.ptr(self.row_scale[s0:s1]), _lib.stream()),
                               "mdir_pack_stats_i8")
                else:
                    _lib.check(lib.mdir_pack_stats(_lib.ptr(self.db32[s0:s1]), _lib.ptr(self.db16[s0:s1]), m, self.D, _lib.ptr(st),
                                                   _lib.stream()), "mdir_pack_stats")
                torch.maximum(self._stats, st, out=self._stats)
            self._n_used = s1
            self._set_live(np.arange(s0, s1, dtype=np.int64), 1)
            return torch.arange(self.idx_base + s0, self.idx_base + s1, dtype=torch.int64)

    @contextlib.contextmanager
    def _live_version(self, live):
        if live is None:
            yield
            return
        cur, self.live = self.live, live
        try:
            yield
        finally:
            self.live = cur

    def stats(self):
        if self._stats is None:
            if self.db32 is None:
                raise _lib.MdirError("the shortlist certificate needs the fp32 master copy (keep_fp32=True)")
            st = torch.zeros((4,), dtype=torch.float32, device=self.device)
            lib = _lib.lib()
            with torch.cuda.device(self.device):
                if self.D % 128 == 0 and self.n >= I8_MIN_ROWS:
                    db8 = torch.empty((self.n, self.D), dtype=torch.int8, device=self.device)
                    rs = torch.empty((self.n,), dtype=torch.float32, device=self.device)
                    _lib.check(lib.mdir_pack_stats_i8(_lib.ptr(self.db32), _lib.ptr(self.db16), self.n, self.D, _lib.ptr(st), _lib.ptr(db8),
                                                      _lib.ptr(rs), _lib.stream()), "mdir_pack_stats_i8")
                    if float(st[3].item()) < I8_MAX_REL_RESIDUAL ** 2:
                        self.db8, self.row_scale = db8, rs
                else:
                    _lib.check(lib.mdir_pack_stats(_lib.ptr(self.db32), _lib.ptr(self.db16), self.n, self.D, _lib.ptr(st), _lib.stream()),
                               "mdir_pack_stats")
            self._stats = st
        return self._stats

    def _buf(self, name, shape, dtype):
        key = (getattr(self, "_ws_tag", None), name, tuple(shape), dtype)
        b = self._ws.get(key)
        if b is None:
            b = torch.empty(shape, dtype=dtype, device=self.device)
            self._ws[key] = b
        return b

    def _plan(self, kth):
        n_tiles = (self.n + TILE - 1) // TILE
        if n_tiles < 64:
            return None
        want = -(-kth * n_tiles // TARGET_CAND)
        if want > 148:
            want = -(-want // 148) * 148
        n_sample = max(32, min(MAX_SAMPLE_TILES, n_tiles // 4, want))
        stride = n_tiles // n_sample
        if n_sample * TILE < 2 * kth or stride < 2:
            return None
        return n_sample, stride

    def _fused_ok(self, kth, nq=1):
        if not self.fused or nq > MAX_Q:
            return False
        n_tiles = (self.n + TILE - 1) // TILE
        if self._sms is None:
            self._sms = torch.cuda.get_device_properties(self.device).multi_processor_count
        g = balanced_grid(n_tiles, min(148, self._sms, n_tiles // 2))
        if n_tiles < 64 or g * 16 < 2 * kth:
            return False
        return 1.25 * kth * n_tiles / (g * g) <= FUSED_CAP_L / 2

    def _i8_route(self, kth, nq):
        if not (self.certify and self.db32 is not None and self.D % 128 == 0 and self._fused_ok(kth, nq)):
            return False
        self.stats()
        return self.db8 is not None

    def _fused_ws(self):
        ws = self._ws.get("fused_ws")
        if ws is None:
            ws = torch.zeros((_lib.lib().mdir_sim_scan_fused_workspace_bytes(MAX_Q) // 4,), dtype=torch.int32, device=self.device)
            self._ws["fused_ws"] = ws
        return ws

    def _topk_block_i8(self, q32, kth, k_out, out_scores, out_idx, out_keys, ovf):
        lib = _lib.lib()
        nq = q32.shape[0]
        n_pad = -(-nq // 16) * 16
        stats = self.stats()
        q8 = self._buf("q8", (2 * n_pad, self.D), torch.int8)
        qsc = self._buf("q8_scale", (nq, 2), torch.float32)
        qeps = self._buf("q8_eps", (nq,), torch.float32)
        _lib.check(lib.mdir_pack_q_i8(_lib.ptr(q32), nq, self.D, _lib.ptr(stats), _lib.ptr(q8), _lib.ptr(qsc), _lib.ptr(qeps), _lib.stream()),
                   "mdir_pack_q_i8")
        tau, cand, cnt = self._cand_bufs(nq)
        ws = self._fused_ws()
        prof = getattr(self, "prof", None)
        if prof is not None:
            prof.begin()
        _lib.check(lib.mdir_sim_scan_fused_i8_live(_lib.ptr(self.db8), _lib.ptr(self.row_scale), self.n, _lib.ptr(q8), _lib.ptr(qsc), nq, self.D,
                                                   kth, _lib.ptr(tau), self.idx_base, _lib.ptr(cand), _lib.ptr(cnt), 0, FUSED_CAP_L, _lib.ptr(ws),
                                                   _lib.ptr(self.live), _lib.stream()), "mdir_sim_scan_fused_i8_live")
        if prof is not None:
            prof.end(self.n * self.D + 4 * self.n)
        self._finalize(cand, cnt, nq, kth, out_scores, out_idx, out_keys, tau, ovf, (q32, k_out), caps=(0, FUSED_CAP_L), q_eps=qeps)

    def _scan(self, q16, mode, stride, n_sample, dense, dense_ld, tau, cand, cnt):
        fn = _lib.lib().mdir_sim_scan_wide_bf16_live if q16.shape[0] > MAX_Q else _lib.lib().mdir_sim_scan_bf16_live
        _lib.check(fn(_lib.ptr(self.db16), self.n, _lib.ptr(q16), q16.shape[0], self.D, mode, stride,
                      n_sample, _lib.ptr(dense), dense_ld, _lib.ptr(tau), self.idx_base, _lib.ptr(cand),
                      _lib.ptr(cnt), CAP_S, CAP_L, _lib.ptr(self.live), _lib.stream()), "mdir_sim_scan_bf16_live")

    def _cand_bufs(self, nq=MAX_Q_WIDE):
        rows = MAX_Q_WIDE if nq <= MAX_Q_WIDE else WIDE_Q
        return (self._buf("tau", (rows,), torch.int64), self._buf("cand", (rows, CAND_ROW), torch.int64),
                self._buf("segcnt", (rows, N_SEGS), torch.int32))

    def _finalize(self, cand, cnt, nq, kth, out_scores, out_idx, out_keys, tau, ovf, rescore=None, caps=(CAP_S, CAP_L), q_eps=None):
        CAP_S, CAP_L = caps
        CAND_ROW = CAP_S + 148 * CAP_L
        if rescore is None:
            _lib.check(_lib.lib().mdir_topk_finalize(_lib.ptr(cand), CAND_ROW, _lib.ptr(cnt), N_SEGS, CAP_S, CAP_L, nq, kth,
                                                     _lib.ptr(out_scores), _lib.ptr(out_idx), _lib.ptr(out_keys), _lib.ptr(tau),
                                                     _lib.ptr(ovf), _lib.stream()), "mdir_topk_finalize")
        elif q_eps is not None:
            q32, k_out = rescore
            _lib.check(_lib.lib().mdir_topk_finalize_rescore_eps(_lib.ptr(cand), CAND_ROW, _lib.ptr(cnt), N_SEGS, CAP_S, CAP_L, nq, kth, k_out,
                                                                 _lib.ptr(self.db32), self.n, self.idx_base, _lib.ptr(q32), self.D,
                                                                 _lib.ptr(self.stats()), _lib.ptr(q_eps), _lib.ptr(out_scores), _lib.ptr(out_idx),
                                                                 _lib.ptr(out_keys), _lib.ptr(tau), _lib.ptr(ovf), _lib.stream()),
                       "mdir_topk_finalize_rescore_eps")
        else:
            q32, k_out = rescore
            stats = self.stats() if self.certify else None
            _lib.check(_lib.lib().mdir_topk_finalize_rescore(_lib.ptr(cand), CAND_ROW, _lib.ptr(cnt), N_SEGS, CAP_S, CAP_L, nq, kth, k_out,
                                                             _lib.ptr(self.db32), self.n, self.idx_base, _lib.ptr(q32), self.D,
                                                             _lib.ptr(stats), _lib.ptr(out_scores), _lib.ptr(out_idx), _lib.ptr(out_keys),
                                                             _lib.ptr(tau), _lib.ptr(ovf), _lib.stream()), "mdir_topk_finalize_rescore")

    def _dense_block(self, q16, kth, out_scores, out_idx, out_keys, ovf, rescore=None):
        lib = _lib.lib()
        nq = q16.shape[0]
        tau, cand, cnt = self._cand_bufs(nq)
        dense = self._buf("dense", (MAX_Q if nq <= MAX_Q else (MAX_Q_WIDE if nq <= MAX_Q_WIDE else WIDE_Q), max(self.n, 1)), torch.float32)
        self._scan(q16, 0, 0, 0, dense, self.n, None, None, None)
        _lib.check(lib.mdir_select_kth_live(_lib.ptr(dense), self.n, self.n, nq, kth, 0, self.idx_base, _lib.ptr(tau), _lib.ptr(cand),
                                            CAND_ROW, _lib.ptr(cnt), N_SEGS, CAP_S, 0, _lib.ptr(self.live), _lib.stream()), "mdir_select_kth_live")
        self._finalize(cand, cnt, nq, kth, out_scores, out_idx, out_keys, tau, ovf, rescore)

    def _topk_block(self, q16, kth, out_scores, out_idx, out_keys, ovf, rescore=None):
        lib = _lib.lib()
        nq = q16.shape[0]
        plan = self._plan(kth)
        if plan is None:
            return self._dense_block(q16, kth, out_scores, out_idx, out_keys, ovf, rescore)
        tau, cand, cnt = self._cand_bufs(nq)
        prof = getattr(self, "prof", None)
        if self._fused_ok(kth, nq):
            ws = self._fused_ws()
            if prof is not None:
                prof.begin()
            _lib.check(lib.mdir_sim_scan_fused_bf16_live(_lib.ptr(self.db16), self.n, _lib.ptr(q16), nq, self.D, kth, _lib.ptr(tau),
                                                         self.idx_base, _lib.ptr(cand), _lib.ptr(cnt), 0, FUSED_CAP_L, _lib.ptr(ws),
                                                         _lib.ptr(self.live), _lib.stream()), "mdir_sim_scan_fused_bf16_live")
            if prof is not None:
                prof.end(self.n * self.D * 2)
            return self._finalize(cand, cnt, nq, kth, out_scores, out_idx, out_keys, tau, ovf, rescore, caps=(0, FUSED_CAP_L))
        n_sample, stride = plan
        rows = n_sample * TILE
        if nq <= MAX_Q_WIDE:
            sample = self._buf("sample", (MAX_Q if nq <= MAX_Q else MAX_Q_WIDE, MAX_SAMPLE_TILES * TILE), torch.float32)
            ld = MAX_SAMPLE_TILES * TILE
        else:
            sample = self._buf("sample_wide", (WIDE_Q, rows), torch.float32)
            ld = rows
        self._scan(q16, 1, stride, n_sample, sample, ld, None, None, None)
        _lib.check(lib.mdir_select_kth_live(_lib.ptr(sample), ld, rows, nq, kth, stride, self.idx_base, _lib.ptr(tau), _lib.ptr(cand),
                                            CAND_ROW, _lib.ptr(cnt), N_SEGS, CAP_S, 1, _lib.ptr(self.live), _lib.stream()), "mdir_select_kth_live")
        if prof is not None:
            prof.begin()
        self._scan(q16, 2, stride, n_sample, None, 0, tau, cand, cnt)
        if prof is not None:
            prof.end((self.n - rows) * self.D * 2)
        self._finalize(cand, cnt, nq, kth, out_scores, out_idx, out_keys, tau, ovf, rescore)

    def search(self, q, k, precision="fp32", shortlist=None, check=True, return_keys=False, block_q=MAX_Q):
        lib = _lib.lib()
        with torch.cuda.device(self.device):
            q32 = _as_dev_f32(q, self.device)
            nq_all = q32.shape[0]
            if q32.shape[1] != self.D:
                raise _lib.MdirError("query dimension %d != database dimension %d" % (q32.shape[1], self.D))
            k = int(k)
            if nq_all == 0:
                empty = (torch.empty((0, k), dtype=torch.float32, device=self.device), torch.empty((0, k), dtype=torch.int32, device=self.device))
                return empty + (torch.empty((0, k), dtype=torch.int64, device=self.device),) if return_keys else empty
            k_eff = min(k, self.n)
            if precision == "fp32":
                if self.db32 is None:
                    raise _lib.MdirError("precision='fp32' needs keep_fp32=True")
                kth = max(k_eff, min(self.n, int(shortlist or default_shortlist(k))))
            elif precision == "bf16":
                kth = k_eff
            else:
                raise ValueError("precision must be 'fp32' or 'bf16'")
            if kth > 4096:
                raise _lib.MdirError("k/shortlist %d too large for the fused path (max 4096); use ranks()" % kth)
            q16 = None
            out_s = torch.empty((nq_all, k), dtype=torch.float32, device=self.device)
            out_i = torch.empty((nq_all, k), dtype=torch.int32, device=self.device)
            out_k = torch.empty((nq_all, k), dtype=torch.int64, device=self.device) if return_keys else None
            self._ovf = self._buf("ovf", (max(nq_all, 1),), torch.int32)
            block_q = max(MAX_Q, min(WIDE_Q, int(block_q)))
            for q0 in range(0, nq_all, block_q):
                q1 = min(q0 + block_q, nq_all)
                nq = q1 - q0
                ovf = self._ovf[q0:q1]
                bs, bi = out_s[q0:q1], out_i[q0:q1]
                bk = out_k[q0:q1] if return_keys else None
                rescore = (q32[q0:q1], k_eff) if precision == "fp32" else None
                kk = kth if precision == "fp32" else k_eff
                qb = None
                if rescore is None or not self._i8_route(kk, nq):
                    if q16 is None:
                        q16 = pack_bf16(q32)
                    qb = q16[q0:q1]
                if k_eff < k:
                    bs.fill_(float("-inf")); bi.fill_(-1)
                    if bk is not None:
                        bk.fill_(-1)
                    tmp_s = torch.empty((nq, k_eff), dtype=torch.float32, device=self.device)
                    tmp_i = torch.empty((nq, k_eff), dtype=torch.int32, device=self.device)
                    tmp_k = torch.empty((nq, k_eff), dtype=torch.int64, device=self.device)
                    self._run_block(qb, kk, tmp_s, tmp_i, tmp_k, ovf, check, rescore=rescore)
                    bs[:, :k_eff] = tmp_s; bi[:, :k_eff] = tmp_i
                    if bk is not None:
                        bk[:, :k_eff] = tmp_k
                else:
                    self._run_block(qb, kk, bs, bi, bk, ovf, check, rescore=rescore)
            if return_keys:
                return out_s, out_i, out_k
            return out_s, out_i

    def _run_block(self, q16, kth, out_s, out_i, out_k, ovf, check, rescore=None):
        if q16 is None:
            self.route = "int8"
            self.cert["int8_blocks"] += 1
            self._topk_block_i8(rescore[0], kth, rescore[1], out_s, out_i, out_k, ovf)
            if not check:
                return
            st = ovf.cpu()
            if not bool(st.any()):
                self.cert["queries"] += int(st.numel())
                return
            self.cert["int8_redone"] += 1
            q16 = pack_bf16(rescore[0])
        self.route = "bf16"
        self._topk_block(q16, kth, out_s, out_i, out_k, ovf, rescore)
        if not check:
            return
        st = ovf.cpu()
        self.cert["queries"] += int(st.numel())
        if bool((st & STATUS_OVERFLOW).any()):
            self._dense_block(q16, kth, out_s, out_i, out_k, ovf, rescore)
            st = ovf.cpu()
            if bool((st & STATUS_OVERFLOW).any()):
                raise _lib.MdirError("dense recovery overflowed (internal error)")
        if rescore is None:
            return
        self.cert["flagged"] += int((st & STATUS_UNCERTIFIED).ne(0).sum())
        k_max = min(self.n, MAX_KTH)
        while bool((st & STATUS_UNCERTIFIED).any()) and kth < k_max:
            kth = min(2 * kth, k_max)
            self.cert["widened_blocks"] += 1
            self._topk_block(q16, kth, out_s, out_i, out_k, ovf, rescore)
            st = ovf.cpu()
            if bool((st & STATUS_OVERFLOW).any()):
                self._dense_block(q16, kth, out_s, out_i, out_k, ovf, rescore)
                st = ovf.cpu()
        self.cert["uncertified"] += int((st & STATUS_UNCERTIFIED).ne(0).sum())

    def check_overflow(self):
        return bool(self._ovf.any().item())

    def status(self):
        return self._ovf

    def _split3(self, x, role):
        n, D = x.shape
        out = torch.empty((n, 3 * D), dtype=torch.float32, device=self.device)
        _lib.check(_lib.lib().mdir_split_tf32x3(_lib.ptr(x), n, D, role, _lib.ptr(out), _lib.stream()), "mdir_split_tf32x3")
        return out

    def scores(self, q, out=None, precision="bf16"):
        self._require_all_live("Index.scores()")
        lib = _lib.lib()
        with torch.cuda.device(self.device):
            q32 = _as_dev_f32(q, self.device)
            nq_all = q32.shape[0]
            if out is None:
                out = torch.empty((nq_all, self.n), dtype=torch.float32, device=self.device)
            if precision == "bf16":
                q16 = pack_bf16(q32)
                if nq_all > MAX_Q and out.stride(0) >= self.n and self.n > 0:
                    for q0 in range(0, nq_all, DENSE_LAUNCH_Q):
                        q1 = min(q0 + DENSE_LAUNCH_Q, nq_all)
                        _lib.check(lib.mdir_sim_scan_dense_bf16(_lib.ptr(self.db16), self.n, _lib.ptr(q16[q0:q1]), q1 - q0, self.D,
                                                                _lib.ptr(out[q0:q1]), out.stride(0), _lib.stream()), "mdir_sim_scan_dense_bf16")
                    return out
                for q0 in range(0, nq_all, MAX_Q):
                    q1 = min(q0 + MAX_Q, nq_all)
                    self._scan(q16[q0:q1], 0, 0, 0, out[q0:q1], out.stride(0), None, None, None)
                return out
            if precision not in ("tf32", "fp32"):
                raise ValueError("precision must be 'bf16', 'tf32' or 'fp32'")
            if self.db32 is None:
                raise _lib.MdirError("precision=%r needs keep_fp32=True" % precision)
            if precision == "tf32":
                dbx, qx, D = self.db32, q32, self.D
            else:
                if getattr(self, "_db_x3", None) is None:
                    self._db_x3 = self._split3(self.db32, 0)
                dbx, qx, D = self._db_x3, self._split3(q32, 1), 3 * self.D
            for q0 in range(0, nq_all, MAX_Q):
                q1 = min(q0 + MAX_Q, nq_all)
                _lib.check(lib.mdir_sim_scan_tf32(_lib.ptr(dbx), self.n, _lib.ptr(qx[q0:q1]), q1 - q0, D, 0, 0, 0, _lib.ptr(out[q0:q1]),
                                                  self.n, None, self.idx_base, None, None, 0, 0, _lib.stream()), "mdir_sim_scan_tf32")
            return out

    def ranks(self, q, max_pairs=1 << 28, precision="bf16"):
        self._require_all_live("Index.ranks()")
        lib = _lib.lib()
        with torch.cuda.device(self.device):
            q32 = _as_dev_f32(q, self.device)
            nq_all = q32.shape[0]
            out = torch.empty((self.n, nq_all), dtype=torch.int64, device=self.device)
            if nq_all == 0 or self.n == 0:
                return out
            chunk = max(1, min(nq_all, max_pairs // max(self.n, 1)))
            chunk = max(1, min(chunk, 65535))
            ws = _rank_workspace(self.n, chunk, self.device)
            sc = torch.empty((chunk, self.n), dtype=torch.float32, device=self.device)
            starts = list(range(0, nq_all, chunk))
            status = torch.zeros((len(starts),), dtype=torch.int32, device=self.device)
            for c, q0 in enumerate(starts):
                q1 = min(q0 + chunk, nq_all)
                self.scores(q32[q0:q1], out=sc[:q1 - q0], precision=precision)
                _lib.check(lib.mdir_rank_scores_hist(_lib.ptr(sc), self.n, q1 - q0, 1, _lib.ptr(out[:, q0:]), nq_all, _lib.ptr(ws),
                                                     _lib.ptr(status[c:]), _lib.stream()), "mdir_rank_scores_hist")
            RANK_STATS["fast"] += len(starts)
            for c, st in enumerate(status.cpu().tolist()):
                if not st:
                    continue
                q0 = starts[c]
                q1 = min(q0 + chunk, nq_all)
                self.scores(q32[q0:q1], out=sc[:q1 - q0], precision=precision)
                _rank_scores_slow(sc, self.n, q1 - q0, 1, out[:, q0:], nq_all, ws, st)
            return out


RANK_STATS = {"fast": 0, "sample_sort": 0, "fallback": 0}


def _rank_workspace(n_db, n_q, device):
    lib = _lib.lib()
    return torch.empty(max(lib.mdir_rank_workspace_bytes(n_db, n_q), lib.mdir_rank_fast_workspace_bytes(n_db, n_q),
                           lib.mdir_rank_hist_workspace_bytes(n_db, n_q)) + 256,
                       dtype=torch.uint8, device=device)


def _rank_scores_slow(scores, n_db, n_q, query_major, out, out_ld, ws, status):
    lib = _lib.lib()
    if status & 2:
        RANK_STATS["sample_sort"] += 1
        st = torch.empty((1,), dtype=torch.int32, device=scores.device)
        _lib.check(lib.mdir_rank_scores_fast(_lib.ptr(scores), n_db, n_q, query_major, _lib.ptr(out), out_ld, _lib.ptr(ws), _lib.ptr(st),
                                             _lib.stream()), "mdir_rank_scores_fast")
        status = int(st.item())
    if status & 1:
        RANK_STATS["fallback"] += 1
        _lib.check(lib.mdir_rank_scores(_lib.ptr(scores), n_db, n_q, query_major, _lib.ptr(out), out_ld, _lib.ptr(ws), _lib.stream()),
                   "mdir_rank_scores")


def _rank_scores(scores, n_db, n_q, query_major, out, out_ld, ws):
    lib = _lib.lib()
    status = torch.empty((1,), dtype=torch.int32, device=scores.device)
    _lib.check(lib.mdir_rank_scores_hist(_lib.ptr(scores), n_db, n_q, query_major, _lib.ptr(out), out_ld, _lib.ptr(ws), _lib.ptr(status),
                                         _lib.stream()), "mdir_rank_scores_hist")
    RANK_STATS["fast"] += 1
    st = int(status.item())
    if st:
        _rank_scores_slow(scores, n_db, n_q, query_major, out, out_ld, ws, st)


def ranks_from_scores(scores, device="cuda", method="auto"):
    lib = _lib.lib()
    dev = torch.device(device)
    s = _as_dev_f32(scores, dev)
    n_db, n_q = s.shape
    with torch.cuda.device(dev):
        out = torch.empty((n_db, n_q), dtype=torch.int64, device=dev)
        if n_db == 0 or n_q == 0:
            return out
        for q0 in range(0, n_q, 65535):
            q1 = min(n_q, q0 + 65535)
            blk = s if (q0 == 0 and q1 == n_q) else s[:, q0:q1].contiguous()
            ws = _rank_workspace(n_db, q1 - q0, dev)
            if method == "radix":
                _lib.check(lib.mdir_rank_scores(_lib.ptr(blk), n_db, q1 - q0, 0, _lib.ptr(out[:, q0:]), n_q, _lib.ptr(ws), _lib.stream()),
                           "mdir_rank_scores")
            else:
                _rank_scores(blk, n_db, q1 - q0, 0, out[:, q0:], n_q, ws)
    return out


def topk_from_scores(scores, k, device="cuda"):
    lib = _lib.lib()
    dev = torch.device(device)
    s = _as_dev_f32(scores, dev)
    n_db, n_q = s.shape
    k = int(k)
    if k > min(n_db, 4096):
        r = ranks_from_scores(s, device=dev)[:k]
        return r, torch.gather(s, 0, r)
    cap = int(min(STAGE_CAP, max(4 * k, 1024)))
    with torch.cuda.device(dev):
        st = s.t().contiguous()
        tau = torch.empty((n_q,), dtype=torch.int64, device=dev)
        cand = torch.empty((n_q, cap), dtype=torch.int64, device=dev)
        cnt = torch.zeros((n_q,), dtype=torch.int32, device=dev)
        out_s = torch.empty((n_q, k), dtype=torch.float32, device=dev)
        out_i = torch.empty((n_q, k), dtype=torch.int32, device=dev)
        _lib.check(lib.mdir_select_kth(_lib.ptr(st), n_db, n_db, n_q, k, 0, 0, _lib.ptr(tau), _lib.ptr(cand), cap, _lib.ptr(cnt), 1, cap, 0,
                                       _lib.stream()), "mdir_select_kth")
        _lib.check(lib.mdir_topk_finalize(_lib.ptr(cand), cap, _lib.ptr(cnt), 1, cap, 0, n_q, k, _lib.ptr(out_s), _lib.ptr(out_i), None,
                                          None, None, _lib.stream()), "mdir_topk_finalize")
        if int(cnt.max().item()) > cap:
            r = ranks_from_scores(s, device=dev)[:k]
            return r, torch.gather(s, 0, r)
    return out_i.t().contiguous().long(), out_s.t().contiguous()


def rank(vecs, qvecs, device="cuda", precision="fp32"):
    dev = torch.device(device)
    index = Index(vecs, dxn=True, device=dev, keep_fp32=(precision != "bf16"))
    q = _as_dev_f32(qvecs, dev).t().contiguous()
    return index.ranks(q, precision=precision).cpu().numpy()


class ShardedIndex:

    p2p = True
    P2P_MAX_Q, P2P_MAX_K = 128, 1024

    def __init__(self, local_vecs, idx_base, group=None, device="cuda", keep_fp32=True, dxn=False):
        import torch.distributed as dist
        self.dist = dist
        self.group = group
        self.world = dist.get_world_size(group) if dist.is_initialized() else 1
        self.local = Index(local_vecs, dxn=dxn, device=device, keep_fp32=keep_fp32, idx_base=idx_base)
        self.device = self.local.device
        self._p2p_setup()

    @classmethod
    def from_local(cls, local_index, group=None):
        import torch.distributed as dist
        self = cls.__new__(cls)
        self.dist = dist
        self.group = group
        self.world = dist.get_world_size(group) if dist.is_initialized() else 1
        self.local = local_index
        self.device = local_index.device
        self._p2p_setup()
        return self

    def _p2p_setup(self):
        self._mb, self._mb_own, self._mb_keep = None, None, None
        dist = self.dist
        if not (self.p2p and self.world > 1 and self.world <= 16 and self.device.type == "cuda" and dist.get_backend(self.group) == "nccl"):
            return
        import ctypes as C
        lib = _lib.lib()
        rank = dist.get_rank(self.group)
        ok = 1
        own = C.c_void_p(0)
        handle = (C.c_ubyte * 64)()
        with torch.cuda.device(self.device):
            nbytes = lib.mdir_shard_mailbox_bytes(self.world, self.P2P_MAX_Q, self.P2P_MAX_K)
            if lib.mdir_p2p_alloc(nbytes, C.byref(own), handle) != 0:
                ok = 0
            mine = torch.tensor(list(bytes(handle)) + [ok], dtype=torch.uint8, device=self.device)
            allh = torch.empty((self.world, 65), dtype=torch.uint8, device=self.device)
            dist.all_gather_into_tensor(allh.view(-1), mine, group=self.group)
            allh = allh.cpu().numpy()
            ptrs = (C.c_void_p * self.world)()
            good = bool(allh[:, 64].all())
            if good:
                for r in range(self.world):
                    if r == rank:
                        ptrs[r] = own.value
                        continue
                    peer = C.c_void_p(0)
                    hb = (C.c_ubyte * 64)(*[int(x) for x in allh[r, :64]])
                    if lib.mdir_p2p_open(hb, C.byref(peer)) != 0:
                        good = False
                        break
                    ptrs[r] = peer.value
            flag = torch.tensor([1 if good else 0], dtype=torch.int32, device=self.device)
            dist.all_reduce(flag, op=dist.ReduceOp.MIN, group=self.group)
            if int(flag.item()) == 1:
                self._mb, self._mb_own, self._rank = ptrs, own, rank
            torch.cuda.synchronize(self.device)

    def close(self):
        if self._mb is None:
            return
        lib = _lib.lib()
        torch.cuda.synchronize(self.device)
        self.dist.barrier(group=self.group)
        for r in range(self.world):
            if r != self._rank:
                lib.mdir_p2p_close(self._mb[r])
        lib.mdir_p2p_free(self._mb_own)
        self._mb, self._mb_own = None, None

    def exchange_status(self):
        if self._mb is None:
            return 0
        import ctypes as C
        st = C.c_int(0)
        _lib.check(_lib.lib().mdir_shard_status(self._mb_own, C.byref(st)), "mdir_shard_status")
        return int(st.value)

    @staticmethod
    def shard_bounds(n_total, world, rank):
        per = (n_total + world - 1) // world
        lo = min(rank * per, n_total)
        return lo, min(lo + per, n_total)

    def _id_ranges(self):
        if getattr(self, "_ranges", None) is None:
            loc = self.local
            if self.world == 1:
                self._ranges = [(loc.idx_base, loc.idx_base + loc.n)]
            else:
                dev = self.device if self.dist.get_backend(self.group) == "nccl" else torch.device("cpu")
                mine = torch.tensor([loc.idx_base, loc.idx_base + loc.n], dtype=torch.int64, device=dev)
                allr = torch.empty((self.world * 2,), dtype=torch.int64, device=dev)
                self.dist.all_gather_into_tensor(allr, mine, group=self.group)
                r = allr.cpu().tolist()
                self._ranges = [(int(r[2 * i]), int(r[2 * i + 1])) for i in range(self.world)]
        return self._ranges

    def _local_ids(self, ids):
        rank = self.dist.get_rank(self.group) if self.world > 1 else 0
        return ids_for_rank(ids, self._id_ranges(), rank)

    def remove(self, ids):
        self.local.remove(self._local_ids(ids))

    def restore(self, ids):
        self.local.restore(self._local_ids(ids))

    def search(self, q, k, precision="fp32", shortlist=None, check=True, exchange="sync"):
        s, i, keys = self.local.search(q, k, precision=precision, shortlist=shortlist, check=check, return_keys=True)
        nq_all = keys.shape[0]
        local_status = self.local._ovf[:nq_all]
        if self.world == 1:
            self._status = local_status
            return s, i
        if exchange not in ("sync", "deferred"):
            raise ValueError("exchange must be 'sync' or 'deferred'")
        if self._mb is None or k > self.P2P_MAX_K:
            if exchange == "deferred":
                raise _lib.MdirError("exchange='deferred' needs the peer-memory mailboxes (and k <= %d)" % self.P2P_MAX_K)
            bits = torch.stack([local_status & STATUS_OVERFLOW, local_status & STATUS_UNCERTIFIED])
            if nq_all:
                self.dist.all_reduce(bits, op=self.dist.ReduceOp.MAX, group=self.group)
            self._status = bits[0] | bits[1]
            return merge_keys(keys, self.world, self.group, k)
        if exchange == "deferred" and nq_all > self.P2P_MAX_Q:
            raise _lib.MdirError("exchange='deferred' handles at most %d queries per call" % self.P2P_MAX_Q)
        out_s = torch.empty((nq_all, k), dtype=torch.float32, device=self.device)
        out_i = torch.empty((nq_all, k), dtype=torch.int32, device=self.device)
        self._status = torch.empty((max(nq_all, 1),), dtype=torch.int32, device=self.device)[:nq_all]
        for q0 in range(0, nq_all, self.P2P_MAX_Q):
            q1 = min(q0 + self.P2P_MAX_Q, nq_all)
            self._exchange(keys[q0:q1], q1 - q0, k, 1 if exchange == "deferred" else 0, out_s[q0:q1], out_i[q0:q1],
                           local_status[q0:q1], self._status[q0:q1])
        return out_s, out_i

    def status(self):
        return self._status

    def check_overflow(self):
        return bool(self._status.any().item())

    def search_collective_recovery(self, q, k, precision="fp32", shortlist=None):
        s, i, keys = self.local.search(q, k, precision=precision, shortlist=shortlist, check=True, return_keys=True)
        if self.world == 1:
            return s, i
        return merge_keys(keys, self.world, self.group, k)

    def _exchange(self, keys, nq, k, mode, out_s, out_i, local_status=None, out_status=None):
        import ctypes as C
        with torch.cuda.device(self.device):
            _lib.check(_lib.lib().mdir_shard_exchange_merge(_lib.ptr(keys), nq, k, self._rank, self.world, self.P2P_MAX_Q, self.P2P_MAX_K, mode,
                                                            C.cast(self._mb, C.c_void_p), _lib.ptr(out_s), _lib.ptr(out_i),
                                                            _lib.ptr(local_status), _lib.ptr(out_status), _lib.stream()),
                       "mdir_shard_exchange_merge")

    def drain(self, n_q, k, out=None, status=None):
        if out is None:
            out = (torch.empty((n_q, k), dtype=torch.float32, device=self.device), torch.empty((n_q, k), dtype=torch.int32, device=self.device))
        if status is None:
            status = torch.empty((n_q,), dtype=torch.int32, device=self.device)
        self._status = status
        self._exchange(None, n_q, k, 2, out[0], out[1], None, status)
        return out


def merge_keys(local_keys, world, group, k):
    import torch.distributed as dist
    lib = _lib.lib()
    nq = local_keys.shape[0]
    gathered = torch.empty((world * nq, k), dtype=torch.int64, device=local_keys.device)
    dist.all_gather_into_tensor(gathered, local_keys.contiguous(), group=group)
    allk = gathered.view(world, nq, k).permute(1, 0, 2).contiguous().view(nq, world * k)
    cnt = torch.full((nq,), world * k, dtype=torch.int32, device=local_keys.device)
    out_s = torch.empty((nq, k), dtype=torch.float32, device=local_keys.device)
    out_i = torch.empty((nq, k), dtype=torch.int32, device=local_keys.device)
    with torch.cuda.device(local_keys.device):
        _lib.check(lib.mdir_topk_finalize(_lib.ptr(allk), world * k, _lib.ptr(cnt), 1, world * k, 0, nq, k, _lib.ptr(out_s), _lib.ptr(out_i),
                                          None, None, None, _lib.stream()), "mdir_topk_finalize")
    return out_s, out_i



def make_keys_host(scores, idx):
    s = np.ascontiguousarray(scores, dtype=np.float32).copy()
    s[s == 0] = 0.0
    u = s.view(np.uint32)
    o = np.where(u >> 31 != 0, ~u, u | np.uint32(0x80000000)).astype(np.uint32)
    d = np.where(np.isnan(s), np.uint32(0xffffffff), ~o).astype(np.uint32)
    return (d.astype(np.uint64) << np.uint64(32)) | np.asarray(idx).astype(np.uint32).astype(np.uint64)


def keys_to_host(keys):
    keys = np.asarray(keys).astype(np.uint64)
    o = (~(keys >> np.uint64(32))).astype(np.uint32)
    u = np.where(o >> 31 != 0, o & np.uint32(0x7fffffff), ~o).astype(np.uint32)
    sc = u.view(np.float32).copy()
    idx = (keys & np.uint64(0xffffffff)).astype(np.int64)
    pad = keys == np.uint64(0xffffffffffffffff)
    sc[pad] = -np.inf
    idx[pad] = -1
    return sc, idx


def merge_keys_host(gathered, k):
    g = np.asarray(gathered).astype(np.uint64)
    world, nq, kk = g.shape
    allk = np.transpose(g, (1, 0, 2)).reshape(nq, world * kk)
    return np.sort(allk, axis=1)[:, :k]


def merge_keys_by_rank_host(gathered, k):
    g = np.asarray(gathered).astype(np.uint64)
    world, nq, kk = g.shape
    pad = np.uint64(0xffffffffffffffff)
    out = np.full((nq, k), pad, dtype=np.uint64)
    for q in range(nq):
        for r in range(world):
            for j in range(kk):
                key = g[r, q, j]
                if key == pad:
                    continue
                pos = j
                for o in range(world):
                    if o != r:
                        pos += int(np.searchsorted(g[o, q], key, side="left"))
                if pos < k:
                    out[q, pos] = key
    return out


class GraphedSearch:

    def __init__(self, index, n_q, k, precision="fp32", shortlist=None, prof=None, deferred=False, overlap=False, split=False,
                 scan_ctas=0, fin_chunk=0, fin_stage=0):
        self.index = index
        self.local = index.local if isinstance(index, ShardedIndex) else index
        dev = self.local.device
        self.n_q, self.k, self.precision, self.shortlist = int(n_q), int(k), precision, shortlist
        sharded = isinstance(index, ShardedIndex) and index.world > 1
        self._has_exchange = sharded
        self.overlap = bool(overlap) and sharded and index._mb is not None and self.k <= index.P2P_MAX_K and self.n_q <= index.P2P_MAX_Q
        self.deferred = bool(deferred) and sharded and not self.overlap
        self.q = torch.zeros((n_q, self.local.D), dtype=torch.float32, device=dev)
        self.local.prof = None
        extra = {"exchange": "deferred"} if self.deferred else {}
        k_eff = min(self.k, self.local.n)
        self.kth = max(k_eff, min(self.local.n, int(shortlist or default_shortlist(self.k))))
        self.split = (bool(split) and (self.overlap or (bool(overlap) and not sharded)) and precision == "fp32" and self.local.db32 is not None
                      and k_eff == self.k and self.n_q <= MAX_Q and self.local._fused_ok(self.kth, self.n_q))
        if self.split and not sharded:
            self.overlap = True
        self.scan_ctas, self.fin_chunk, self.fin_stage = int(scan_ctas), int(fin_chunk), int(fin_stage)
        if self.split:
            self._init_split(prof)
            return

        def step():
            if self.overlap:
                return self.local.search(self.q, self.k, precision=self.precision, shortlist=self.shortlist, check=False, return_keys=True)
            return index.search(self.q, self.k, precision=self.precision, shortlist=self.shortlist, check=False, **extra)

        with torch.cuda.device(dev):
            side = torch.cuda.Stream(device=dev)
            side.wait_stream(torch.cuda.current_stream(dev))
            with torch.cuda.stream(side):
                for _ in range(3):
                    step()
            torch.cuda.current_stream(dev).wait_stream(side)
            torch.cuda.synchronize(dev)
            self.local.prof = prof
            self.graph = torch.cuda.CUDAGraph()
            with torch.cuda.graph(self.graph):
                res = step()
                self.ovf = self.local._ovf[:n_q].clone()
                if self.overlap:
                    self.keys = res[2]
                    self.out = (torch.empty((n_q, self.k), dtype=torch.float32, device=dev), torch.empty((n_q, self.k), dtype=torch.int32, device=dev))
                    self.status = torch.zeros((n_q,), dtype=torch.int32, device=dev)
                else:
                    self.out = res
                    self.status = index._status[:n_q].clone() if sharded else self.ovf
            self.local.prof = None
            if self.overlap:
                self.local_done, self.done = torch.cuda.Event(), torch.cuda.Event()

    def _init_split(self, prof):
        loc, dev, nq, k = self.local, self.local.device, self.n_q, self.k
        lib = _lib.lib()
        loc._ws_tag = ("graph", id(self))
        try:
            tau, cand, cnt = loc._cand_bufs(nq)
            ovf = loc._buf("ovf", (max(nq, 1),), torch.int32)
        finally:
            loc._ws_tag = None
        ws = loc._fused_ws()
        i8 = loc._i8_route(self.kth, nq)
        if i8:
            stats = loc.stats()
            self.q8 = torch.empty((2 * (-(-nq // 16) * 16), loc.D), dtype=torch.int8, device=dev)
            self.q8_scale = torch.empty((nq, 2), dtype=torch.float32, device=dev)
            self.q8_eps = torch.empty((nq,), dtype=torch.float32, device=dev)
        else:
            self.q16 = torch.empty((nq, loc.D), dtype=torch.bfloat16, device=dev)
        self.keys = torch.empty((nq, k), dtype=torch.int64, device=dev)
        self.local_out = (torch.empty((nq, k), dtype=torch.float32, device=dev), torch.empty((nq, k), dtype=torch.int32, device=dev))
        self.ovf = ovf[:nq]
        if self._has_exchange:
            self.out = (torch.empty((nq, k), dtype=torch.float32, device=dev), torch.empty((nq, k), dtype=torch.int32, device=dev))
            self.status = torch.zeros((nq,), dtype=torch.int32, device=dev)
        else:
            self.out, self.status = self.local_out, self.ovf

        def front():
            if i8:
                _lib.check(lib.mdir_pack_q_i8(_lib.ptr(self.q), nq, loc.D, _lib.ptr(stats), _lib.ptr(self.q8), _lib.ptr(self.q8_scale),
                                              _lib.ptr(self.q8_eps), _lib.stream()), "mdir_pack_q_i8")
            else:
                _lib.check(lib.mdir_pack_bf16(_lib.ptr(self.q), nq, loc.D, 0, _lib.ptr(self.q16), _lib.stream()), "mdir_pack_bf16")
            if prof is not None:
                prof.begin()
            lib.mdir_tune(1, self.scan_ctas)
            try:
                if i8:
                    _lib.check(lib.mdir_sim_scan_fused_i8_live(_lib.ptr(loc.db8), _lib.ptr(loc.row_scale), loc.n, _lib.ptr(self.q8),
                                                               _lib.ptr(self.q8_scale), nq, loc.D, self.kth, _lib.ptr(tau), loc.idx_base, _lib.ptr(cand),
                                                               _lib.ptr(cnt), 0, FUSED_CAP_L, _lib.ptr(ws), _lib.ptr(loc.live), _lib.stream()),
                               "mdir_sim_scan_fused_i8_live")
                else:
                    _lib.check(lib.mdir_sim_scan_fused_bf16_live(_lib.ptr(loc.db16), loc.n, _lib.ptr(self.q16), nq, loc.D, self.kth, _lib.ptr(tau),
                                                                 loc.idx_base, _lib.ptr(cand), _lib.ptr(cnt), 0, FUSED_CAP_L, _lib.ptr(ws),
                                                                 _lib.ptr(loc.live), _lib.stream()), "mdir_sim_scan_fused_bf16_live")
            finally:
                lib.mdir_tune(1, 0)
            if prof is not None:
                prof.end(loc.n * loc.D + 4 * loc.n if i8 else loc.n * loc.D * 2)

        def back():
            chunk = self.fin_chunk if self.fin_chunk > 0 else nq
            lib.mdir_tune(2, 0 if self.fin_chunk > 0 else 1)
            lib.mdir_tune(3, self.fin_stage)
            try:
                for q0 in range(0, nq, chunk):
                    q1 = min(q0 + chunk, nq)
                    loc._finalize(cand[q0:q1], cnt[q0:q1], q1 - q0, self.kth, self.local_out[0][q0:q1], self.local_out[1][q0:q1],
                                  self.keys[q0:q1], tau[q0:q1], self.ovf[q0:q1], (self.q[q0:q1], k), caps=(0, FUSED_CAP_L),
                                  q_eps=self.q8_eps[q0:q1] if i8 else None)
            finally:
                lib.mdir_tune(2, 1)
                lib.mdir_tune(3, 0)
            if self._has_exchange:
                self.index._exchange(self.keys, nq, k, 0, self.out[0], self.out[1], self.ovf, self.status)

        with torch.cuda.device(dev):
            side = torch.cuda.Stream(device=dev)
            side.wait_stream(torch.cuda.current_stream(dev))
            with torch.cuda.stream(side):
                for _ in range(2):
                    front()
                    back()
            torch.cuda.current_stream(dev).wait_stream(side)
            torch.cuda.synchronize(dev)
            self.graph, self.back = torch.cuda.CUDAGraph(), torch.cuda.CUDAGraph()
            with torch.cuda.graph(self.graph):
                front()
            with torch.cuda.graph(self.back):
                back()
            self.local_done, self.done = torch.cuda.Event(), torch.cuda.Event()

    def exchange(self):
        if getattr(self, "split", False):
            self.back.replay()
            return
        if self._has_exchange:
            self.index._exchange(self.keys, self.n_q, self.k, 0, self.out[0], self.out[1], self.ovf, self.status)

    def __call__(self, q=None):
        if q is not None:
            self.q.copy_(q, non_blocking=True)
        self.graph.replay()
        if self.overlap:
            self.exchange()
        return self.out

    def drain(self):
        if self.deferred:
            self.index.drain(self.n_q, self.k, out=self.out, status=self.status)
        return self.out

    def check_overflow(self):
        return bool(self.status.any().item())


class SearchPipeline:

    def __init__(self, index, n_q, k, depth=None, precision="fp32", shortlist=None, prof=None, deferred=None, overlap=None, split=True,
                 scan_ctas=None):
        self.index = index
        self.local = index.local if isinstance(index, ShardedIndex) else index
        dev = self.local.device
        self.n_q, self.k = int(n_q), int(k)
        self.precision, self.shortlist = precision, shortlist
        sharded = isinstance(index, ShardedIndex) and index.world > 1
        p2p_ok = sharded and index._mb is not None and self.k <= index.P2P_MAX_K and self.n_q <= index.P2P_MAX_Q
        if overlap is None:
            overlap = p2p_ok and not deferred
        self.overlap = bool(overlap) and p2p_ok
        if deferred is None:
            deferred = False
        self.deferred = bool(deferred) and p2p_ok and not self.overlap
        single_split = (not sharded) and split == "single" and overlap is not False and not deferred
        if scan_ctas is None:
            scan_ctas = SINGLE_GPU_SCAN_CTAS if single_split else 0
        n_graphs = int(depth) if depth else (3 if (self.deferred or self.overlap or single_split) else 2)
        self.graphs = [GraphedSearch(index, n_q, k, precision=precision, shortlist=shortlist, prof=prof if s == 0 else None,
                                     deferred=self.deferred, overlap=self.overlap or single_split, split=split, scan_ctas=scan_ctas)
                       for s in range(n_graphs)]
        if single_split:
            self.overlap = all(g.split for g in self.graphs)
        self.depth = n_graphs
        with torch.cuda.device(dev):
            self.compute, self.h2d, self.d2h, self.exch = (torch.cuda.Stream(device=dev) for _ in range(4))
            self.slots = []
            for _ in range(self.depth):
                self.slots.append({
                    "scores": torch.empty((self.n_q, self.k), dtype=torch.float32).pin_memory(),
                    "idx": torch.empty((self.n_q, self.k), dtype=torch.int32).pin_memory(),
                    "ovf": torch.zeros((self.n_q,), dtype=torch.int32).pin_memory(),
                    "up": torch.cuda.Event(), "done": torch.cuda.Event(), "down": torch.cuda.Event(), "local": torch.cuda.Event(),
                    "q": None, "pending": False, "merged": False, "used": False, "live": None})
            if self.deferred:
                self.drain_out = (torch.empty((self.n_q, self.k), dtype=torch.float32, device=dev),
                                  torch.empty((self.n_q, self.k), dtype=torch.int32, device=dev))
                self.drain_status = torch.zeros((self.n_q,), dtype=torch.int32, device=dev)
                with torch.cuda.stream(self.compute):
                    index.drain(self.n_q, self.k, out=self.drain_out, status=self.drain_status)
            torch.cuda.synchronize(dev)
        self.n_submitted = 0
        self.n_recovered = 0

    def _mutate(self, fn):
        dev = self.local.device
        with torch.cuda.device(dev):
            if self.overlap:
                self.compute.wait_stream(self.exch)
            with torch.cuda.stream(self.compute):
                waiting = [sl for sl in self.slots if sl["pending"] and sl["live"] is None]
                if waiting:
                    snap = self.local.live.clone()
                    for sl in waiting:
                        sl["live"] = snap
                return fn()

    def remove(self, ids):
        self._mutate(lambda: self.index.remove(ids))

    def restore(self, ids):
        self._mutate(lambda: self.index.restore(ids))

    def add(self, vecs):
        if isinstance(self.index, ShardedIndex):
            raise _lib.MdirError("SearchPipeline.add() needs an Index: ShardedIndex has no add()")
        return self._mutate(lambda: self.index.add(vecs))

    def _download(self, slot, src, status):
        with torch.cuda.stream(self.d2h):
            slot["scores"].copy_(src[0], non_blocking=True)
            slot["idx"].copy_(src[1], non_blocking=True)
            slot["ovf"].copy_(status, non_blocking=True)
            slot["down"].record()
        slot["merged"] = True

    def submit(self, q):
        t_new = self.n_submitted
        slot, gs = self.slots[t_new % self.depth], self.graphs[t_new % self.depth]
        if slot["pending"]:
            raise _lib.MdirError("SearchPipeline: collect result() of ticket %d before submitting more" % (t_new - self.depth))
        q = torch.as_tensor(q)
        if tuple(q.shape) != tuple(gs.q.shape):
            raise _lib.MdirError("SearchPipeline expects query batches of shape %s" % (tuple(gs.q.shape),))
        with torch.cuda.stream(self.h2d):
            gs.q.copy_(q, non_blocking=True)
            slot["up"].record()
        with torch.cuda.stream(self.compute):
            self.compute.wait_event(slot["up"])
            if self.overlap and slot["used"]:
                self.compute.wait_event(slot["done"])
            gs.graph.replay()
            if self.overlap:
                slot["local"].record()
            else:
                slot["done"].record()
        if self.overlap:
            with torch.cuda.stream(self.exch):
                self.exch.wait_event(slot["local"])
                gs.exchange()
                slot["done"].record()
        slot["q"], slot["pending"], slot["merged"], slot["used"] = q, True, False, True
        self.d2h.wait_event(slot["done"])
        if not self.deferred:
            self._download(slot, gs.out, gs.status)
        elif t_new >= 1 and self.slots[(t_new - 1) % self.depth]["pending"]:
            self._download(self.slots[(t_new - 1) % self.depth], gs.out, gs.status)
        self.n_submitted += 1
        return t_new

    def result(self, ticket):
        if not (self.n_submitted - self.depth <= ticket < self.n_submitted):
            raise _lib.MdirError("SearchPipeline: ticket %d is not in flight" % ticket)
        slot = self.slots[ticket % self.depth]
        if not slot["pending"]:
            raise _lib.MdirError("SearchPipeline: result(%d) was already collected" % ticket)
        if not slot["merged"]:
            if ticket != self.n_submitted - 1:
                raise _lib.MdirError("SearchPipeline: collect deferred results in submission order")
            with torch.cuda.stream(self.compute):
                self.index.drain(self.n_q, self.k, out=self.drain_out, status=self.drain_status)
                ev = torch.cuda.Event()
                ev.record()
            self.d2h.wait_event(ev)
            self._download(slot, self.drain_out, self.drain_status)
        slot["down"].synchronize()
        slot["pending"] = False
        if bool(slot["ovf"].any()):
            self.n_recovered += 1
            sharded = isinstance(self.index, ShardedIndex) and self.index.world > 1
            if sharded and bool((slot["ovf"] & STATUS_PEER_TIMEOUT).any()):
                raise _lib.MdirError("SearchPipeline: a peer rank did not deliver its keys for ticket %d within the bounded wait" % ticket)
            if self.overlap:
                self.compute.wait_stream(self.exch)
            with torch.cuda.stream(self.compute), self.local._live_version(slot["live"]):
                if sharded:
                    s, i = self.index.search_collective_recovery(slot["q"], self.k, precision=self.precision, shortlist=self.shortlist)
                else:
                    s, i = self.index.search(slot["q"], self.k, precision=self.precision, shortlist=self.shortlist)
                slot["scores"].copy_(s)
                slot["idx"].copy_(i)
            self.compute.synchronize()
        slot["q"], slot["live"] = None, None
        return slot["scores"].numpy(), slot["idx"].numpy()

    def map(self, batches):
        tickets = []
        for q in batches:
            if len(tickets) == self.depth:
                yield self.result(tickets.pop(0))
            tickets.append(self.submit(q))
        for t in tickets:
            yield self.result(t)
```

Before: 115,200.

## Tighten int8 rescore band with per-row error bounds

Computes a per-row int8 quantization error norm at pack time and per-query coefficients at query pack, then uses them in finalize to shrink the epsilon band per candidate. The goal is fewer rows sent to fp32 rescoring in the finalize kernel while keeping the ranking certified. It also lowers the int8 route threshold from 900k to 500k rows and replaces single-row rescoring with the two-row path. This adds an extra row_err gather per band candidate and a new n_n rescored output.

```diff
diff --git a/include/mdir_b200.h b/include/mdir_b200.h
--- a/include/mdir_b200.h
+++ b/include/mdir_b200.h
@@ -8,7 +8,7 @@
 extern "C" {
 #endif
 
-#define MDIR_ABI_VERSION 3
+#define MDIR_ABI_VERSION 4
 
 #define MDIR_E_ARG      (-1)
 #define MDIR_E_DRIVER   (-2)
@@ -156,16 +156,24 @@
                                    const float* db_stats, const float* q_eps,
                                    float* out_scores, int32_t* out_idx, uint64_t* out_keys,
                                    uint64_t* tau, int32_t* overflow, void* stream);
+int mdir_topk_finalize_rescore_rowbound(const uint64_t* cand, int64_t cand_row, const uint32_t* seg_counts, int n_seg,
+                                        int cap0, int cap_l, int n_q, int shortlist, int k_out,
+                                        const float* db32, int64_t n_db, uint32_t idx_base, const float* q32, int D,
+                                        const float* db_stats, const float* q_eps, const float* row_err,
+                                        const float* q_ab, float* out_scores, int32_t* out_idx, uint64_t* out_keys,
+                                        uint64_t* tau, int32_t* overflow, int32_t* n_rescored, void* stream);
 #define MDIR_STATUS_OVERFLOW    1
 #define MDIR_STATUS_UNCERTIFIED 2
 
 int mdir_pack_stats(const float* db32, const uint16_t* db16, int64_t n, int D, float* stats, void* stream);
 
 int mdir_pack_stats_i8(const float* db32, const uint16_t* db16, int64_t n, int D, float* stats,
-                       int8_t* db8, float* row_scale, void* stream);
+                       int8_t* db8, float* row_scale, float* row_err, void* stream);
 
 int mdir_pack_q_i8(const float* q32, int n_q, int D, const float* stats, int8_t* q8, float* q_scale,
                    float* q_eps, void* stream);
+int mdir_pack_q_i8_ab(const float* q32, int n_q, int D, const float* stats, int8_t* q8, float* q_scale,
+                      float* q_eps, float* q_ab, void* stream);
 
 int mdir_rescore_f32(const float* db32, int64_t n_db, uint32_t idx_base, const float* q32, int n_q, int D,
                      const int32_t* idx, int kk, uint64_t* out_keys, void* stream);
diff --git a/mdir_b200/_lib.py b/mdir_b200/_lib.py
--- a/mdir_b200/_lib.py
+++ b/mdir_b200/_lib.py
@@ -4,7 +4,7 @@
 _HERE = os.path.dirname(os.path.abspath(__file__))
 LIB_PATH = os.path.join(_HERE, "libmdir_b200.so")
 _lib = None
-ABI_VERSION = 3
+ABI_VERSION = 4
 
 
 class ImageDesc(C.Structure):
@@ -51,9 +51,12 @@
     "mdir_topk_finalize": (_i, [_vp, _i64, _vp, _i, _i, _i, _i, _i, _vp, _vp, _vp, _vp, _vp, _vp]),
     "mdir_topk_finalize_rescore": (_i, [_vp, _i64, _vp, _i, _i, _i, _i, _i, _i, _vp, _i64, _u32, _vp, _i, _vp, _vp, _vp, _vp, _vp, _vp, _vp]),
     "mdir_topk_finalize_rescore_eps": (_i, [_vp, _i64, _vp, _i, _i, _i, _i, _i, _i, _vp, _i64, _u32, _vp, _i, _vp, _vp, _vp, _vp, _vp, _vp, _vp, _vp]),
+    "mdir_topk_finalize_rescore_rowbound": (_i, [_vp, _i64, _vp, _i, _i, _i, _i, _i, _i, _vp, _i64, _u32, _vp, _i, _vp, _vp, _vp, _vp, _vp, _vp,
+                                                 _vp, _vp, _vp, _vp, _vp]),
     "mdir_pack_stats": (_i, [_vp, _vp, _i64, _i, _vp, _vp]),
-    "mdir_pack_stats_i8": (_i, [_vp, _vp, _i64, _i, _vp, _vp, _vp, _vp]),
+    "mdir_pack_stats_i8": (_i, [_vp, _vp, _i64, _i, _vp, _vp, _vp, _vp, _vp]),
     "mdir_pack_q_i8": (_i, [_vp, _i, _i, _vp, _vp, _vp, _vp, _vp]),
+    "mdir_pack_q_i8_ab": (_i, [_vp, _i, _i, _vp, _vp, _vp, _vp, _vp, _vp]),
     "mdir_rescore_f32": (_i, [_vp, _i64, _u32, _vp, _i, _i, _vp, _i, _vp, _vp]),
     "mdir_qe_accumulate": (_i, [_vp, _i64, _u32, _i, _vp, _vp, _i, _i, _f, _vp, _vp]),
     "mdir_add_l2n": (_i, [_vp, _vp, _i, _i, _vp, _vp]),
diff --git a/mdir_b200/csrc/topk.cu b/mdir_b200/csrc/topk.cu
--- a/mdir_b200/csrc/topk.cu
+++ b/mdir_b200/csrc/topk.cu
@@ -468,10 +468,10 @@
         const uint32_t g0 = (uint32_t)key0, g1 = (uint32_t)key1;
         const int64_t row0 = (int64_t)g0 - (int64_t)idx_base, row1 = (int64_t)g1 - (int64_t)idx_base;
         const bool ok0 = key0 != ~0ull && row0 >= 0 && row0 < n_db, ok1 = key1 != ~0ull && row1 >= 0 && row1 < n_db;
-        float s0 = 0.f, s1 = 0.f;
+        float s0 = 0.f, s1 = 0.f, dummy;
         if (ok0 && ok1) rescore_row2(db32 + row0 * D, db32 + row1 * D, qs, D, lane, s0, s1);
-        else if (ok0) s0 = rescore_row(db32 + row0 * D, qs, D, lane);
-        else if (ok1) s1 = rescore_row(db32 + row1 * D, qs, D, lane);
+        else if (ok0) rescore_row2(db32 + row0 * D, db32 + row0 * D, qs, D, lane, s0, dummy);
+        else if (ok1) rescore_row2(db32 + row1 * D, db32 + row1 * D, qs, D, lane, s1, dummy);
         const uint64_t n0 = ok0 ? make_key(s0, g0) : ~0ull, n1 = ok1 ? make_key(s1, g1) : ~0ull;
         __syncwarp();
         if (lane == 0) {
@@ -494,7 +494,9 @@
                                                              uint64_t* __restrict__ tau, int32_t* __restrict__ overflow,
                                                              const float* __restrict__ db32, int64_t n_db, uint32_t idx_base,
                                                              const float* __restrict__ q32, int D, int k_out,
-                                                             const float* __restrict__ db_stats, const float* __restrict__ q_eps) {
+                                                             const float* __restrict__ db_stats, const float* __restrict__ q_eps,
+                                                             const float* __restrict__ row_err, const float* __restrict__ q_ab,
+                                                             int32_t* __restrict__ n_rescored) {
     extern __shared__ uint64_t skeys[];
     __shared__ uint32_t hist[256];
     __shared__ uint64_t s_prefix;
@@ -718,11 +720,39 @@
             const uint64_t tkey = s_tkey;
             const uint64_t bound = tkey == ~0ull ? ~0ull : ((uint64_t)desc_key(key_score(tkey) - eps) << 32) | 0xffffffffull;
             const int ext_cap = sl_cap - nk;
-            for (int i = threadIdx.x; i < cnt; i += blockDim.x) {
-                const uint64_t key = skeys[i];
-                if (key > last16 && key <= bound && key != ~0ull) {
-                    const uint32_t pos = atomicAdd(&s_out, 1u);
-                    if (pos < (uint32_t)ext_cap) sl[nk + pos] = key;
+            if (row_err && tkey != ~0ull) {
+                const float t = key_score(tkey), a_q = q_ab[2 * q], b_q = q_ab[2 * q + 1];
+                constexpr int kPer = 4;
+                for (int i0 = 0; i0 < cnt; i0 += kPer * 1024) {
+                    uint64_t keys[kPer];
+                    float err[kPer];
+#pragma unroll
+                    for (int u = 0; u < kPer; ++u) {
+                        const int i = i0 + threadIdx.x + u * 1024;
+                        keys[u] = i < cnt ? skeys[i] : ~0ull;
+                        const int64_t row = (int64_t)(uint32_t)keys[u] - (int64_t)idx_base;
+                        const bool band = keys[u] > last16 && keys[u] <= bound && keys[u] != ~0ull;
+                        err[u] = band && row >= 0 && row < n_db ? row_err[row] : INFINITY;
+                    }
+#pragma unroll
+                    for (int u = 0; u < kPer; ++u) {
+                        if (keys[u] > last16 && keys[u] <= bound && keys[u] != ~0ull) {
+                            const float eps_r = fminf(eps, fmaf(err[u], a_q, b_q) * 1.001f + 1e-7f);
+                            const uint64_t bound_r = ((uint64_t)desc_key(t - eps_r) << 32) | 0xffffffffull;
+                            if (keys[u] <= bound_r) {
+                                const uint32_t pos = atomicAdd(&s_out, 1u);
+                                if (pos < (uint32_t)ext_cap) sl[nk + pos] = keys[u];
+                            }
+                        }
+                    }
+                }
+            } else {
+                for (int i = threadIdx.x; i < cnt; i += blockDim.x) {
+                    const uint64_t key = skeys[i];
+                    if (key > last16 && key <= bound && key != ~0ull) {
+                        const uint32_t pos = atomicAdd(&s_out, 1u);
+                        if (pos < (uint32_t)ext_cap) sl[nk + pos] = key;
+                    }
                 }
             }
             __syncthreads();
@@ -758,6 +788,7 @@
         }
         nres = n_all;
         k_emit = k_out;
+        if (threadIdx.x == 0 && n_rescored) n_rescored[q] = n_all;
     }
     if (threadIdx.x == 0 && overflow) overflow[q] = status;
     for (int j = threadIdx.x; j < k_emit; j += blockDim.x) {
@@ -926,7 +957,8 @@
 static int launch_finalize(const uint64_t* cand, int64_t cand_row, const uint32_t* seg_counts, int n_seg, int cap0, int cap_l, int n_q,
                            int k, float* out_scores, int32_t* out_idx, uint64_t* out_keys, uint64_t* tau, int32_t* overflow,
                            const float* db32, int64_t n_db, uint32_t idx_base, const float* q32, int D, int k_out, const float* db_stats,
-                           void* stream, const float* q_eps = nullptr) {
+                           void* stream, const float* q_eps = nullptr, const float* row_err = nullptr, const float* q_ab = nullptr,
+                           int32_t* n_rescored = nullptr) {
     MDIR_CHECK_ARG(cand && seg_counts && n_seg >= 1 && n_seg <= MDIR_CAND_SEGS && cap0 >= 0 && n_q >= 0 && k >= 1 && k <= 4096);
     MDIR_CHECK_ARG(n_seg == 1 || cap_l >= 1);
     MDIR_CHECK_ARG(cand_row >= (int64_t)cap0 + (int64_t)(n_seg - 1) * cap_l);
@@ -973,13 +1005,14 @@
         cfg.attrs = attr;
         cfg.numAttrs = 1;
         MDIR_CUDA(cudaLaunchKernelEx(&cfg, topk_finalize_kernel<2>, cand, cand_row, seg_counts, n_seg, cap0, cap_l, k, smem_cap, sl_cap, out_scores,
-                                     out_idx, out_keys, tau, overflow, db32, n_db, idx_base, q32, D, k_out, db_stats, q_eps));
+                                     out_idx, out_keys, tau, overflow, db32, n_db, idx_base, q32, D, k_out, db_stats, q_eps,
+                                     row_err, q_ab, n_rescored));
         MDIR_LAUNCH_CHECK();
         return 0;
     }
     topk_finalize_kernel<1><<<n_q, 1024, smem, (cudaStream_t)stream>>>(cand, cand_row, seg_counts, n_seg, cap0, cap_l, k, smem_cap, sl_cap,
                                                                         out_scores, out_idx, out_keys, tau, overflow, db32, n_db, idx_base,
-                                                                        q32, D, k_out, db_stats, q_eps);
+                                                                        q32, D, k_out, db_stats, q_eps, row_err, q_ab, n_rescored);
     MDIR_LAUNCH_CHECK();
     return 0;
 }
@@ -1000,14 +1033,24 @@
                            db32, n_db, idx_base, q32, D, k_out, db_stats, stream);
 }
 
+extern "C" int mdir_topk_finalize_rescore_rowbound(const uint64_t* cand, int64_t cand_row, const uint32_t* seg_counts, int n_seg,
+                                                   int cap0, int cap_l, int n_q, int shortlist, int k_out, const float* db32, int64_t n_db,
+                                                   uint32_t idx_base, const float* q32, int D, const float* db_stats, const float* q_eps,
+                                                   const float* row_err, const float* q_ab, float* out_scores, int32_t* out_idx,
+                                                   uint64_t* out_keys, uint64_t* tau, int32_t* overflow, int32_t* n_rescored, void* stream) {
+    MDIR_CHECK_ARG(db32 != nullptr && db_stats != nullptr && q_eps != nullptr && (row_err == nullptr || q_ab != nullptr));
+    return launch_finalize(cand, cand_row, seg_counts, n_seg, cap0, cap_l, n_q, shortlist, out_scores, out_idx, out_keys, tau, overflow,
+                           db32, n_db, idx_base, q32, D, k_out, db_stats, stream, q_eps, row_err, q_ab, n_rescored);
+}
+
 extern "C" int mdir_topk_finalize_rescore_eps(const uint64_t* cand, int64_t cand_row, const uint32_t* seg_counts, int n_seg, int cap0,
                                               int cap_l, int n_q, int shortlist, int k_out, const float* db32, int64_t n_db,
                                               uint32_t idx_base, const float* q32, int D, const float* db_stats, const float* q_eps,
                                               float* out_scores, int32_t* out_idx, uint64_t* out_keys, uint64_t* tau, int32_t* overflow,
                                               void* stream) {
-    MDIR_CHECK_ARG(db32 != nullptr && db_stats != nullptr && q_eps != nullptr);
-    return launch_finalize(cand, cand_row, seg_counts, n_seg, cap0, cap_l, n_q, shortlist, out_scores, out_idx, out_keys, tau, overflow,
-                           db32, n_db, idx_base, q32, D, k_out, db_stats, stream, q_eps);
+    return mdir_topk_finalize_rescore_rowbound(cand, cand_row, seg_counts, n_seg, cap0, cap_l, n_q, shortlist, k_out, db32, n_db, idx_base,
+                                               q32, D, db_stats, q_eps, nullptr, nullptr, out_scores, out_idx, out_keys, tau, overflow,
+                                               nullptr, stream);
 }
 
 namespace mdir {
@@ -1054,7 +1097,7 @@
 
 __global__ void __launch_bounds__(256) pack_stats_i8_kernel(const float* __restrict__ db32, const __nv_bfloat16* __restrict__ db16, int64_t n,
                                                             int D, uint32_t* __restrict__ stats, int8_t* __restrict__ db8,
-                                                            float* __restrict__ row_scale) {
+                                                            float* __restrict__ row_scale, float* __restrict__ row_err) {
     const int lane = threadIdx.x & 31;
     const int64_t warps = (int64_t)gridDim.x * (blockDim.x >> 5);
     float e_max = 0.f, x_max = 0.f, e8_max = 0.f, rel_max = 0.f;
@@ -1083,7 +1126,10 @@
             q2 = fmaf(d0, d0, fmaf(d1, d1, fmaf(d2, d2, fmaf(d3, d3, q2))));
         }
         q2 = warp_sum(q2);
-        if (lane == 0) row_scale[r] = s;
+        if (lane == 0) {
+            row_scale[r] = s;
+            row_err[r] = sqrtf(q2 * 1.001f);
+        }
         e_max = fmaxf(e_max, e2);
         x_max = fmaxf(x_max, x2);
         e8_max = fmaxf(e8_max, q2);
@@ -1098,7 +1144,8 @@
 }
 
 __global__ void __launch_bounds__(32) pack_q_i8_kernel(const float* __restrict__ q32, int n_q, int n_pad, int D, const float* __restrict__ stats,
-                                                       int8_t* __restrict__ q8, float* __restrict__ q_scale, float* __restrict__ q_eps) {
+                                                       int8_t* __restrict__ q8, float* __restrict__ q_scale, float* __restrict__ q_eps,
+                                                       float* __restrict__ q_ab) {
     const int q = blockIdx.x, lane = threadIdx.x;
     int8_t* hi_row = q8 + (int64_t)q * D;
     int8_t* lo_row = q8 + (int64_t)(n_pad + q) * D;
@@ -1151,30 +1198,40 @@
         q_scale[2 * q] = s_hi;
         q_scale[2 * q + 1] = s_lo;
         q_eps[q] = eps * 1.001f + 1e-7f;
+        if (q_ab) {
+            q_ab[2 * q] = sqrtf(qh2);
+            q_ab[2 * q + 1] = x_max * sqrtf(d2) + 1.25f * (float)D * u * x_max * sqrtf(q2) +
+                              8.f * u * (x_max + e8) * (s_hi * sqrtf(h2) + s_lo * sqrtf(l2));
+        }
     }
 }
 }
 
 extern "C" int mdir_pack_stats_i8(const float* db32, const uint16_t* db16, int64_t n, int D, float* stats, int8_t* db8, float* row_scale,
-                                  void* stream) {
-    MDIR_CHECK_ARG(db32 && db16 && stats && db8 && row_scale && n >= 0 && D > 0 && D % 128 == 0);
+                                  float* row_err, void* stream) {
+    MDIR_CHECK_ARG(db32 && db16 && stats && db8 && row_scale && row_err && n >= 0 && D > 0 && D % 128 == 0);
     MDIR_CHECK_ARG((((uintptr_t)db32 | (uintptr_t)db8) & 15) == 0);
     MDIR_CUDA(cudaMemsetAsync(stats, 0, 4 * sizeof(float), (cudaStream_t)stream));
     if (n == 0) return 0;
     const int64_t blocks = (n + 7) / 8;
     pack_stats_i8_kernel<<<(unsigned)(blocks < 148 * 8 ? blocks : 148 * 8), 256, 0, (cudaStream_t)stream>>>(
-        db32, reinterpret_cast<const __nv_bfloat16*>(db16), n, D, reinterpret_cast<uint32_t*>(stats), db8, row_scale);
+        db32, reinterpret_cast<const __nv_bfloat16*>(db16), n, D, reinterpret_cast<uint32_t*>(stats), db8, row_scale, row_err);
     MDIR_LAUNCH_CHECK();
     return 0;
 }
 
-extern "C" int mdir_pack_q_i8(const float* q32, int n_q, int D, const float* stats, int8_t* q8, float* q_scale, float* q_eps, void* stream) {
+extern "C" int mdir_pack_q_i8_ab(const float* q32, int n_q, int D, const float* stats, int8_t* q8, float* q_scale, float* q_eps,
+                                 float* q_ab, void* stream) {
     MDIR_CHECK_ARG(q32 && stats && q8 && q_scale && q_eps && n_q >= 1 && n_q <= 128 && D > 0 && D % 128 == 0);
     MDIR_CHECK_ARG((((uintptr_t)q32 | (uintptr_t)q8) & 15) == 0);
     const int n_pad = (n_q + 15) & ~15;
-    pack_q_i8_kernel<<<n_pad, 32, 0, (cudaStream_t)stream>>>(q32, n_q, n_pad, D, stats, q8, q_scale, q_eps);
+    pack_q_i8_kernel<<<n_pad, 32, 0, (cudaStream_t)stream>>>(q32, n_q, n_pad, D, stats, q8, q_scale, q_eps, q_ab);
     MDIR_LAUNCH_CHECK();
     return 0;
+}
+
+extern "C" int mdir_pack_q_i8(const float* q32, int n_q, int D, const float* stats, int8_t* q8, float* q_scale, float* q_eps, void* stream) {
+    return mdir_pack_q_i8_ab(q32, n_q, D, stats, q8, q_scale, q_eps, nullptr, stream);
 }
 
 extern "C" int mdir_rescore_f32(const float* db32, int64_t n_db, uint32_t idx_base, const float* q32, int n_q, int D,
diff --git a/mdir_b200/search.py b/mdir_b200/search.py
--- a/mdir_b200/search.py
+++ b/mdir_b200/search.py
@@ -24,7 +24,7 @@
 STATUS_OVERFLOW, STATUS_UNCERTIFIED, STATUS_PEER_TIMEOUT = 1, 2, 4
 MAX_KTH = 4096
 I8_MAX_REL_RESIDUAL = 0.02
-I8_MIN_ROWS = 900000
+I8_MIN_ROWS = 500000
 
 
 def default_shortlist(k):
@@ -127,7 +127,7 @@
             self._init_live(n)
         self._ws = {}
         self._stats = None
-        self.db8 = self.row_scale = None
+        self.db8 = self.row_scale = self.row_err = None
         self.route = None
         self.cert = {"queries": 0, "flagged": 0, "widened_blocks": 0, "uncertified": 0, "int8_blocks": 0, "int8_redone": 0}
 
@@ -143,7 +143,7 @@
             self._init_live(self.n)
         self._ws = {}
         self._stats = None
-        self.db8 = self.row_scale = None
+        self.db8 = self.row_scale = self.row_err = None
         self.route = None
         self.cert = {"queries": 0, "flagged": 0, "widened_blocks": 0, "uncertified": 0, "int8_blocks": 0, "int8_redone": 0}
         return self
@@ -207,8 +207,8 @@
                 st = torch.zeros((4,), dtype=torch.float32, device=self.device)
                 if self.db8 is not None:
                     _lib.check(lib.mdir_pack_stats_i8(_lib.ptr(self.db32[s0:s1]), _lib.ptr(self.db16[s0:s1]), m, self.D, _lib.ptr(st),
-                                                      _lib.ptr(self.db8[s0:s1]), _lib.ptr(self.row_scale[s0:s1]), _lib.stream()),
-                               "mdir_pack_stats_i8")
+                                                      _lib.ptr(self.db8[s0:s1]), _lib.ptr(self.row_scale[s0:s1]),
+                                                      _lib.ptr(self.row_err[s0:s1]), _lib.stream()), "mdir_pack_stats_i8")
                 else:
                     _lib.check(lib.mdir_pack_stats(_lib.ptr(self.db32[s0:s1]), _lib.ptr(self.db16[s0:s1]), m, self.D, _lib.ptr(st),
                                                    _lib.stream()), "mdir_pack_stats")
@@ -238,10 +238,11 @@
                 if self.D % 128 == 0 and self.n >= I8_MIN_ROWS:
                     db8 = torch.empty((self.n, self.D), dtype=torch.int8, device=self.device)
                     rs = torch.empty((self.n,), dtype=torch.float32, device=self.device)
+                    re = torch.empty((self.n,), dtype=torch.float32, device=self.device)
                     _lib.check(lib.mdir_pack_stats_i8(_lib.ptr(self.db32), _lib.ptr(self.db16), self.n, self.D, _lib.ptr(st), _lib.ptr(db8),
-                                                      _lib.ptr(rs), _lib.stream()), "mdir_pack_stats_i8")
+                                                      _lib.ptr(rs), _lib.ptr(re), _lib.stream()), "mdir_pack_stats_i8")
                     if float(st[3].item()) < I8_MAX_REL_RESIDUAL ** 2:
-                        self.db8, self.row_scale = db8, rs
+                        self.db8, self.row_scale, self.row_err = db8, rs, re
                 else:
                     _lib.check(lib.mdir_pack_stats(_lib.ptr(self.db32), _lib.ptr(self.db16), self.n, self.D, _lib.ptr(st), _lib.stream()),
                                "mdir_pack_stats")
@@ -301,8 +302,9 @@
         q8 = self._buf("q8", (2 * n_pad, self.D), torch.int8)
         qsc = self._buf("q8_scale", (nq, 2), torch.float32)
         qeps = self._buf("q8_eps", (nq,), torch.float32)
-        _lib.check(lib.mdir_pack_q_i8(_lib.ptr(q32), nq, self.D, _lib.ptr(stats), _lib.ptr(q8), _lib.ptr(qsc), _lib.ptr(qeps), _lib.stream()),
-                   "mdir_pack_q_i8")
+        qab = self._buf("q8_ab", (nq, 2), torch.float32)
+        _lib.check(lib.mdir_pack_q_i8_ab(_lib.ptr(q32), nq, self.D, _lib.ptr(stats), _lib.ptr(q8), _lib.ptr(qsc), _lib.ptr(qeps), _lib.ptr(qab),
+                                         _lib.stream()), "mdir_pack_q_i8_ab")
         tau, cand, cnt = self._cand_bufs(nq)
         ws = self._fused_ws()
         prof = getattr(self, "prof", None)
@@ -313,7 +315,7 @@
                                                    _lib.ptr(self.live), _lib.stream()), "mdir_sim_scan_fused_i8_live")
         if prof is not None:
             prof.end(self.n * self.D + 4 * self.n)
-        self._finalize(cand, cnt, nq, kth, out_scores, out_idx, out_keys, tau, ovf, (q32, k_out), caps=(0, FUSED_CAP_L), q_eps=qeps)
+        self._finalize(cand, cnt, nq, kth, out_scores, out_idx, out_keys, tau, ovf, (q32, k_out), caps=(0, FUSED_CAP_L), q_eps=(qeps, qab))
 
     def _scan(self, q16, mode, stride, n_sample, dense, dense_ld, tau, cand, cnt):
         fn = _lib.lib().mdir_sim_scan_wide_bf16_live if q16.shape[0] > MAX_Q else _lib.lib().mdir_sim_scan_bf16_live
@@ -335,11 +337,13 @@
                                                      _lib.ptr(ovf), _lib.stream()), "mdir_topk_finalize")
         elif q_eps is not None:
             q32, k_out = rescore
-            _lib.check(_lib.lib().mdir_topk_finalize_rescore_eps(_lib.ptr(cand), CAND_ROW, _lib.ptr(cnt), N_SEGS, CAP_S, CAP_L, nq, kth, k_out,
-                                                                 _lib.ptr(self.db32), self.n, self.idx_base, _lib.ptr(q32), self.D,
-                                                                 _lib.ptr(self.stats()), _lib.ptr(q_eps), _lib.ptr(out_scores), _lib.ptr(out_idx),
-                                                                 _lib.ptr(out_keys), _lib.ptr(tau), _lib.ptr(ovf), _lib.stream()),
-                       "mdir_topk_finalize_rescore_eps")
+            eps, ab = q_eps
+            _lib.check(_lib.lib().mdir_topk_finalize_rescore_rowbound(_lib.ptr(cand), CAND_ROW, _lib.ptr(cnt), N_SEGS, CAP_S, CAP_L, nq, kth,
+                                                                      k_out, _lib.ptr(self.db32), self.n, self.idx_base, _lib.ptr(q32), self.D,
+                                                                      _lib.ptr(self.stats()), _lib.ptr(eps), _lib.ptr(self.row_err), _lib.ptr(ab),
+                                                                      _lib.ptr(out_scores), _lib.ptr(out_idx), _lib.ptr(out_keys), _lib.ptr(tau),
+                                                                      _lib.ptr(ovf), None, _lib.stream()),
+                       "mdir_topk_finalize_rescore_rowbound")
         else:
             q32, k_out = rescore
             stats = self.stats() if self.certify else None
@@ -967,6 +971,7 @@
             self.q8 = torch.empty((2 * (-(-nq // 16) * 16), loc.D), dtype=torch.int8, device=dev)
             self.q8_scale = torch.empty((nq, 2), dtype=torch.float32, device=dev)
             self.q8_eps = torch.empty((nq,), dtype=torch.float32, device=dev)
+            self.q8_ab = torch.empty((nq, 2), dtype=torch.float32, device=dev)
         else:
             self.q16 = torch.empty((nq, loc.D), dtype=torch.bfloat16, device=dev)
         self.keys = torch.empty((nq, k), dtype=torch.int64, device=dev)
@@ -980,8 +985,8 @@
 
         def front():
             if i8:
-                _lib.check(lib.mdir_pack_q_i8(_lib.ptr(self.q), nq, loc.D, _lib.ptr(stats), _lib.ptr(self.q8), _lib.ptr(self.q8_scale),
-                                              _lib.ptr(self.q8_eps), _lib.stream()), "mdir_pack_q_i8")
+                _lib.check(lib.mdir_pack_q_i8_ab(_lib.ptr(self.q), nq, loc.D, _lib.ptr(stats), _lib.ptr(self.q8), _lib.ptr(self.q8_scale),
+                                                 _lib.ptr(self.q8_eps), _lib.ptr(self.q8_ab), _lib.stream()), "mdir_pack_q_i8_ab")
             else:
                 _lib.check(lib.mdir_pack_bf16(_lib.ptr(self.q), nq, loc.D, 0, _lib.ptr(self.q16), _lib.stream()), "mdir_pack_bf16")
             if prof is not None:
@@ -1011,7 +1016,7 @@
                     q1 = min(q0 + chunk, nq)
                     loc._finalize(cand[q0:q1], cnt[q0:q1], q1 - q0, self.kth, self.local_out[0][q0:q1], self.local_out[1][q0:q1],
                                   self.keys[q0:q1], tau[q0:q1], self.ovf[q0:q1], (self.q[q0:q1], k), caps=(0, FUSED_CAP_L),
-                                  q_eps=self.q8_eps[q0:q1] if i8 else None)
+                                  q_eps=(self.q8_eps[q0:q1], self.q8_ab[q0:q1]) if i8 else None)
             finally:
                 lib.mdir_tune(2, 1)
                 lib.mdir_tune(3, 0)
```

After: 136,800 (median of 6 runs). 1.19x the previous value.
